# candrewlee14/zgml

Hardware: AMD Instinct MI355X
Metric: decode_tokens_per_sec (higher is better)
Workload: dtype f32; 1 GPU; SmolLM-135M Q4_0 greedy decode, batch 1, 1xMI355X (BASELINE configs[1]); weights=synthetic Q4_0 (int4 + f16 block scale / 32), tied f32 LM head, max_seq=2048, loop=device-resident (inputs in HBM), parallelism=none

## Files before the change

### zgml_amd/csrc/attention_decode.h

```cpp
#pragma once
#include "kernels.h"

#include <hip/hip_fp16.h>
#include <math.h>

namespace zgml {
namespace {

typedef float f4v_t __attribute__((ext_vector_type(4)));
__device__ __forceinline__ float4 ldg4(const float* p) {
    const f4v_t v = *(const __attribute__((address_space(1))) f4v_t*)p;
    return make_float4(v.x, v.y, v.z, v.w);
}
__device__ __forceinline__ float ldg1(const float* p) { return *(const __attribute__((address_space(1))) float*)p; }
__device__ __forceinline__ uint32_t ldgu(const uint32_t* p) { return *(const __attribute__((address_space(1))) uint32_t*)p; }
__device__ __forceinline__ void stg4(float* p, float4 v) { *(__attribute__((address_space(1))) f4v_t*)p = f4v_t{v.x, v.y, v.z, v.w}; }
__device__ __forceinline__ void stg1(float* p, float v) { *(__attribute__((address_space(1))) float*)p = v; }
__device__ __forceinline__ void stgu(uint32_t* p, uint32_t v) { *(__attribute__((address_space(1))) uint32_t*)p = v; }

constexpr int kAttnBlock = 1024;
constexpr int kAttnUnroll = 4;

__device__ __forceinline__ float4 rope4(float4 own, float4 par, float4 c, float4 s, bool is_hi) {
    if (is_hi)
        return make_float4(own.x * c.x + par.x * s.x, own.y * c.y + par.y * s.y, own.z * c.z + par.z * s.z,
                           own.w * c.w + par.w * s.w);
    return make_float4(own.x * c.x - par.x * s.x, own.y * c.y - par.y * s.y, own.z * c.z - par.z * s.z,
                       own.w * c.w - par.w * s.w);
}

__device__ __forceinline__ float score_of(float dot, float mk, float scale) {
    float score = -INFINITY;
    if (isfinite(mk)) {
        score = dot * scale + mk;
        if (!isfinite(score)) score = -INFINITY;
    }
    return score;
}


__device__ __forceinline__ float xor16_sum(float v) {
    auto r = __builtin_amdgcn_permlane16_swap(__float_as_uint(v), __float_as_uint(v), false, false);
    return __uint_as_float(r[0]) + __uint_as_float(r[1]);
}
__device__ __forceinline__ float xor32_sum(float v) {
    auto r = __builtin_amdgcn_permlane32_swap(__float_as_uint(v), __float_as_uint(v), false, false);
    return __uint_as_float(r[0]) + __uint_as_float(r[1]);
}
__device__ __forceinline__ float xor16_max(float v) {
    auto r = __builtin_amdgcn_permlane16_swap(__float_as_uint(v), __float_as_uint(v), false, false);
    return fmaxf(__uint_as_float(r[0]), __uint_as_float(r[1]));
}
__device__ __forceinline__ float xor32_max(float v) {
    auto r = __builtin_amdgcn_permlane32_swap(__float_as_uint(v), __float_as_uint(v), false, false);
    return fmaxf(__uint_as_float(r[0]), __uint_as_float(r[1]));
}

template <int LPK>
__device__ __forceinline__ float group_sum(float v) {
    if (LPK >= 2) v += __int_as_float(__builtin_amdgcn_mov_dpp(__float_as_int(v), 0xB1, 0xF, 0xF, true));
    if (LPK >= 4) v += __int_as_float(__builtin_amdgcn_mov_dpp(__float_as_int(v), 0x4E, 0xF, 0xF, true));
    if (LPK >= 8) v += __int_as_float(__builtin_amdgcn_mov_dpp(__float_as_int(v), 0x141, 0xF, 0xF, true));
    if (LPK >= 16) v += __int_as_float(__builtin_amdgcn_mov_dpp(__float_as_int(v), 0x140, 0xF, 0xF, true));
    if (LPK >= 32) v = xor16_sum(v);
    if (LPK >= 64) v = xor32_sum(v);
    return v;
}

struct SoftState {
    float m, l;
    float4 acc;
};
__device__ __forceinline__ void soft_merge(SoftState& s, float om, float ol, float4 oacc) {
    const float nm = fmaxf(s.m, om);
    const float a = s.m > -INFINITY ? expf(s.m - nm) : 0.0f, b = om > -INFINITY ? expf(om - nm) : 0.0f;
    s.l = s.l * a + ol * b;
    s.acc = make_float4(s.acc.x * a + oacc.x * b, s.acc.y * a + oacc.y * b, s.acc.z * a + oacc.z * b, s.acc.w * a + oacc.w * b);
    s.m = nm;
}

using gu64 = __attribute__((address_space(1))) unsigned long long;
using gu32 = __attribute__((address_space(1))) unsigned int;
__device__ __forceinline__ void split_put(float* p, float a, float b) {
    const unsigned long long v = (unsigned long long)__float_as_uint(a) | ((unsigned long long)__float_as_uint(b) << 32);
    __hip_atomic_store((gu64*)p, v, __ATOMIC_RELAXED, __HIP_MEMORY_SCOPE_AGENT);
// ... 40 lines not shown
__device__ __forceinline__ float row_dot(const float4& q, const AttnRow<false>& r) { return q.x * r.v.x + q.y * r.v.y + q.z * r.v.z + q.w * r.v.w; }
__device__ __forceinline__ float row_dot(const float4& q, const AttnRow<true>& r) {
    const uint32_t kw = r.w;
    return (q.x * (float)(int8_t)(kw & 255) + q.y * (float)(int8_t)((kw >> 8) & 255) + q.z * (float)(int8_t)((kw >> 16) & 255) +
            q.w * (float)(int8_t)(kw >> 24)) * r.sc;
}
__device__ __forceinline__ void row_axpy(float4& acc, float wgt, const AttnRow<false>& r) {
    acc.x += wgt * r.v.x, acc.y += wgt * r.v.y, acc.z += wgt * r.v.z, acc.w += wgt * r.v.w;
}
__device__ __forceinline__ void row_axpy(float4& acc, float wgt, const AttnRow<true>& r) {
    const float ws = wgt * r.sc;
    const uint32_t vw = r.w;
    acc.x += ws * (float)(int8_t)(vw & 255), acc.y += ws * (float)(int8_t)((vw >> 8) & 255);
    acc.z += ws * (float)(int8_t)((vw >> 16) & 255), acc.w += ws * (float)(int8_t)(vw >> 24);
}
__device__ __forceinline__ AttnRow<true> quantise_block32(float4 v) {
    float mx = fmaxf(fmaxf(fabsf(v.x), fabsf(v.y)), fmaxf(fabsf(v.z), fabsf(v.w)));
    mx = fmaxf(mx, __int_as_float(__builtin_amdgcn_mov_dpp(__float_as_int(mx), 0xB1, 0xF, 0xF, true)));
    mx = fmaxf(mx, __int_as_float(__builtin_amdgcn_mov_dpp(__float_as_int(mx), 0x4E, 0xF, 0xF, true)));
    mx = fmaxf(mx, __int_as_float(__builtin_amdgcn_mov_dpp(__float_as_int(mx), 0x141, 0xF, 0xF, true)));
    const float scale = mx > 0.f ? mx / 127.0f : 1.0f, inv = mx > 0.f ? 127.0f / mx : 0.0f;
    auto q8 = [&](float x) { return (uint32_t)(uint8_t)(int8_t)(int)fminf(fmaxf(x * inv, -127.0f), 127.0f); };
    return AttnRow<true>{q8(v.x) | (q8(v.y) << 8) | (q8(v.z) << 16) | (q8(v.w) << 24), scale};
}

#ifndef ZGML_ATTN_KVQ16
#define ZGML_ATTN_KVQ16 1
#endif
constexpr int kAttnUnrollQ16 = 4;
typedef uint32_t u4v_t __attribute__((ext_vector_type(4)));
__device__ __forceinline__ u4v_t ldgu4(const void* p) { return *(const __attribute__((address_space(1))) u4v_t*)p; }
template <int B>
__device__ __forceinline__ float s8_to_f32(uint32_t w) {
    float r;
#if defined(__HIP_DEVICE_COMPILE__)
    if constexpr (B == 0) asm("v_cvt_f32_i32_sdwa %0, sext(%1) dst_sel:DWORD dst_unused:UNUSED_PAD src0_sel:BYTE_0" : "=v"(r) : "v"(w));
    if constexpr (B == 1) asm("v_cvt_f32_i32_sdwa %0, sext(%1) dst_sel:DWORD dst_unused:UNUSED_PAD src0_sel:BYTE_1" : "=v"(r) : "v"(w));
    if constexpr (B == 2) asm("v_cvt_f32_i32_sdwa %0, sext(%1) dst_sel:DWORD dst_unused:UNUSED_PAD src0_sel:BYTE_2" : "=v"(r) : "v"(w));
    if constexpr (B == 3) asm("v_cvt_f32_i32_sdwa %0, sext(%1) dst_sel:DWORD dst_unused:UNUSED_PAD src0_sel:BYTE_3" : "=v"(r) : "v"(w));
#else
    r = (float)(int8_t)(w >> (8 * B));
#endif
    return r;
}
typedef float f32x2_t __attribute__((ext_vector_type(2)));
__device__ __forceinline__ float dot16(const f32x2_t (&q)[8], const u4v_t& w) {
    f32x2_t s = {0.f, 0.f};
#pragma unroll
    for (int c = 0; c < 4; c++) {
        const f32x2_t lo = {s8_to_f32<0>(w[c]), s8_to_f32<1>(w[c])}, hi = {s8_to_f32<2>(w[c]), s8_to_f32<3>(w[c])};
        s = __builtin_elementwise_fma(lo, q[2 * c], s);
        s = __builtin_elementwise_fma(hi, q[2 * c + 1], s);
#if defined(__HIP_DEVICE_COMPILE__)
        __builtin_amdgcn_sched_barrier(0);
#endif
    }
    return s.x + s.y;
}
__device__ __forceinline__ void axpy16(f32x2_t (&acc)[8], float ws, const u4v_t& w) {
    const f32x2_t ws2 = {ws, ws};
#pragma unroll
    for (int c = 0; c < 4; c++) {
        const f32x2_t lo = {s8_to_f32<0>(w[c]), s8_to_f32<1>(w[c])}, hi = {s8_to_f32<2>(w[c]), s8_to_f32<3>(w[c])};
        acc[2 * c] = __builtin_elementwise_fma(lo, ws2, acc[2 * c]);
        acc[2 * c + 1] = __builtin_elementwise_fma(hi, ws2, acc[2 * c + 1]);
#if defined(__HIP_DEVICE_COMPILE__)
        __builtin_amdgcn_sched_barrier(0);
#endif
    }
}
template <int L, bool MAX>
__device__ __forceinline__ float slots_all(float v) {
    auto op = [](float a, float b) { return MAX ? fmaxf(a, b) : a + b; };
    if (L <= 1) v = op(v, __int_as_float(__builtin_amdgcn_mov_dpp(__float_as_int(v), 0x121, 0xF, 0xF, true)));
    if (L <= 2) v = op(v, __int_as_float(__builtin_amdgcn_mov_dpp(__float_as_int(v), 0x122, 0xF, 0xF, true)));
    if (L <= 4) v = op(v, __int_as_float(__builtin_amdgcn_mov_dpp(__float_as_int(v), 0x124, 0xF, 0xF, true)));
    if (L <= 8) v = op(v, __int_as_float(__builtin_amdgcn_mov_dpp(__float_as_int(v), 0x128, 0xF, 0xF, true)));
    if (L <= 16) v = MAX ? xor16_max(v) : xor16_sum(v);
    if (L <= 32) v = MAX ? xor32_max(v) : xor32_sum(v);
    return v;
}

struct DecodeHandoff {
    const uint32_t* cnt;
    uint32_t* seen;
    const uint32_t* idx;
    uint32_t n_heads;
    uint32_t need;
    uint32_t* timeout;
    uint32_t poll_sleep;
};

template <int LPK, bool KVQ, int BLOCK = kAttnBlock>
__device__ __forceinline__ void attention_decode_body(const AttnDecodeParams* __restrict__ params, float* split_buf, uint32_t* split_cnt,
                                                      uint32_t split_min_keys, const uint32_t hx, const uint32_t sp_in, const uint32_t n_sp,
                                                      const DecodeHandoff* ho) {
    constexpr int DH = 4 * LPK, HALF = DH / 2;
    constexpr bool Q16 = KVQ && ZGML_ATTN_KVQ16 != 0 && LPK >= 32;
    constexpr int LPKM = Q16 ? DH / 16 : LPK, KPW = 64 / LPKM, KPW4 = 64 / LPK, U = Q16 ? kAttnUnrollQ16 : kAttnUnroll;
    using Row = AttnRow<KVQ>;
    static_assert(sizeof(AttnDecodeParams) == 248, "the bulk fetch below covers exactly 62 dwords");
    AttnDecodeParams P;
    {
        typedef uint32_t u32x16_t __attribute__((ext_vector_type(16)));
        typedef uint32_t u32x8_t __attribute__((ext_vector_type(8)));
        typedef uint32_t u32x4_t __attribute__((ext_vector_type(4)));
        typedef uint32_t u32x2_t __attribute__((ext_vector_type(2)));
        u32x16_t ra, rb, rc;
        u32x8_t rd;
        u32x4_t re;
        u32x2_t rf;
#if defined(__HIP_DEVICE_COMPILE__)
        const AttnDecodeParams* const rec = params + hx;
        asm volatile("s_load_dwordx16 %0, %6, 0x0\n\ts_load_dwordx16 %1, %6, 0x40\n\ts_load_dwordx16 %2, %6, 0x80\n\t"
                     "s_load_dwordx8 %3, %6, 0xc0\n\ts_load_dwordx4 %4, %6, 0xe0\n\ts_load_dwordx2 %5, %6, 0xf0\n\ts_waitcnt lgkmcnt(0)"
                     : "=&s"(ra), "=&s"(rb), "=&s"(rc), "=&s"(rd), "=&s"(re), "=&s"(rf)
                     : "s"(rec)
                     : "memory");
#else
        ra = rb = rc = u32x16_t{}, rd = u32x8_t{}, re = u32x4_t{}, rf = u32x2_t{};
#endif
        char* const dst = (char*)&P;
        __builtin_memcpy(dst, &ra, 64), __builtin_memcpy(dst + 64, &rb, 64), __builtin_memcpy(dst + 128, &rc, 64);
        __builtin_memcpy(dst + 192, &rd, 32), __builtin_memcpy(dst + 224, &re, 16), __builtin_memcpy(dst + 240, &rf, 8);
    }
    const AttentionParams& p = P.att;
#ifdef ZGML_TRACE
    unsigned long long* const trace = P.trace;
#define ATTN_STAMP(i) do { if (trace && threadIdx.x == 0) trace[i] = wall_clock64(); } while (0)
#else
#define ATTN_STAMP(i) do { } while (0)
#endif
    ATTN_STAMP(0);
    __shared__ __attribute__((aligned(8))) float part_ml[2 * (BLOCK / 64)];
    __shared__ float4 part_acc[(BLOCK / 64) * LPK];
    constexpr int COLV = DH / 4 + DH / 32;
    __shared__ __attribute__((aligned(16))) float q16_lds[Q16 ? DH : 4];
    __shared__ __attribute__((aligned(16))) uint32_t col_lds[Q16 ? 2 * COLV : 4];
    const uint32_t tid = threadIdx.x, lane = tid & 63, w = tid >> 6;
    const uint32_t slot = lane / LPK, li = lane % LPK, d0 = 4 * li, pair = d0 & (HALF - 1);
    const bool is_hi = d0 >= (uint32_t)HALF;
    const uint32_t seq_kv = KVQ ? min(ldgu(p.dyn_seq_kv), P.kvq_cols) : ldgu(p.dyn_seq_kv), dk = ldgu(P.dyn_k_off), dv = ldgu(P.dyn_v_off);
    const uint32_t d2_off = p.dst2 ? ldgu(p.dyn_dst2_off) : 0;
    const bool wait_qkv = ho && ho->cnt;
    float4 q_own, q_par, k_own, k_par, v_new;
    if (!wait_qkv) {
        q_own = ldg4(P.q_src + d0), q_par = ldg4(P.q_src + (d0 ^ HALF));
        k_own = ldg4(P.k_src + d0), k_par = ldg4(P.k_src + (d0 ^ HALF));
        v_new = ldg4(P.v_src + d0);
    }
    const float4 q_c = ldg4(P.q_cs + pair), q_s = ldg4(P.q_cs + HALF + pair);
    const float4 k_c = ldg4(P.k_cs + pair), k_s = ldg4(P.k_cs + HALF + pair);
    ATTN_STAMP(1);
    const uint32_t sp = sp_in;
    uint32_t n_active = 1, k_begin = 0, k_end = seq_kv;
    if (n_sp > 1) {
        n_active = seq_kv / split_min_keys;
        n_active = n_active < 1 ? 1 : (n_active > n_sp ? n_sp : n_active);
        if (sp >= n_active) {
            if (wait_qkv && tid == 0) {
                uint32_t* const seen = ho->seen + (hx * n_sp + sp) * 3;
                seen[0] += ho->need, seen[1] += ho->need, seen[2] += ho->need;
            }
            return;
        }
        const uint32_t chunk = (seq_kv + n_active - 1) / n_active;
        k_begin = min(sp * chunk, seq_kv), k_end = min(k_begin + chunk, seq_kv);
    }
    const uint32_t n_keys = k_end - k_begin;
    constexpr int KEYS_PER_WAVE = Q16 ? KPW : KPW * U;
    uint32_t NW = (n_keys + KEYS_PER_WAVE - 1) / KEYS_PER_WAVE;
    NW = NW < 1 ? 1 : (NW > (uint32_t)(BLOCK / 64) ? (uint32_t)(BLOCK / 64) : NW);
    if (w >= NW) return;
    const uint32_t keys_per_iter = KPW * NW, step_keys = keys_per_iter * U, last = k_end ? k_end - 1 : 0;
    constexpr uint32_t BPC = DH / 32;
    const int8_t* const kq = (const int8_t*)P.k_cache + d0;
    const int8_t* const vq = (const int8_t*)P.v_cache + d0;
    const float* const ksc = P.k_cache + (uint64_t)P.kvq_cols * DH / 4 + d0 / 32;
    const float* const vsc = P.v_cache + (uint64_t)P.kvq_cols * DH / 4 + d0 / 32;
    auto load_k = [&](uint32_t s) -> Row {
        if constexpr (KVQ)
            return Row{ldgu((const uint32_t*)(kq + (uint64_t)s * DH)), ldg1(ksc + (uint64_t)s * BPC)};
        else
            return Row{ldg4(p.k + (uint64_t)s * p.k_cs + d0)};
    };
    auto load_v = [&](uint32_t s) -> Row {
        if constexpr (KVQ)
            return Row{ldgu((const uint32_t*)(vq + (uint64_t)s * DH)), ldg1(vsc + (uint64_t)s * BPC)};
        else
            return Row{ldg4(p.v + (uint64_t)s * p.v_cs + d0)};
    };
    Row kv[Q16 ? 1 : U], vv[Q16 ? 1 : U];
    float mk[U];
    const uint32_t slotm = lane / LPKM, lim = lane % LPKM;
    const char* const kb16 = (const char*)P.k_cache;
    const char* const vb16 = (const char*)P.v_cache;
    const uint32_t sc_base16 = P.kvq_cols * (uint32_t)DH + 4 * (lim / 2);
    u4v_t kw[Q16 ? U : 1], vw[Q16 ? U : 1];
    float ks[Q16 ? U : 1], vs[Q16 ? U : 1];
    auto issue_k16 = [&](uint32_t base) {
#pragma unroll
        for (int j = 0; j < U; j++) {
            const uint32_t s = min(base + j * keys_per_iter + w * KPW + slotm, last);
            kw[j] = ldgu4(kb16 + (s * (uint32_t)DH + 16 * lim));
            ks[j] = ldg1((const float*)(kb16 + (sc_base16 + s * (4 * BPC))));
            mk[j] = ldg1((const float*)((const char*)p.mask + s * (4 * p.mask_rs)));
        }
    };
    auto issue_v16 = [&](uint32_t base) {
#pragma unroll
        for (int j = 0; j < U; j++) {
            const uint32_t s = min(base + j * keys_per_iter + w * KPW + slotm, last);
            vw[j] = ldgu4(vb16 + (s * (uint32_t)DH + 16 * lim));
            vs[j] = ldg1((const float*)(vb16 + (sc_base16 + s * (4 * BPC))));
        }
    };
    if constexpr (Q16) {
        issue_k16(k_begin);
        issue_v16(k_begin);
    } else {
#pragma unroll
        for (int j = 0; j < U; j++) {
            const uint32_t s = min(k_begin + j * keys_per_iter + w * KPW + slot, last);
            kv[j] = load_k(s);
            vv[j] = load_v(s);
            mk[j] = ldg1(p.mask + (uint64_t)s * p.mask_rs);
        }
    }
    uint32_t target[3] = {0, 0, 0};
    if (wait_qkv) {
        const uint32_t ci[3] = {ho->idx[3 * hx], ho->idx[3 * hx + 1], ho->idx[3 * hx + 2]};
        const uint32_t* const seen = ho->seen + (hx * n_sp + sp) * 3;
#pragma unroll
        for (int c = 0; c < 3; c++) target[c] = seen[c] + ho->need;
        if (w == 0) {
            uint32_t spins = 0;
            for (;;) {
                bool ok = true;
#pragma unroll
                for (int c = 0; c < 3; c++)
                    ok = ok && (int32_t)(__hip_atomic_load((gu32*)ho->cnt + 32 * ci[c], __ATOMIC_RELAXED, __HIP_MEMORY_SCOPE_AGENT) - target[c]) >= 0;
                if (ok) break;
                if (++spins > 400000u) {
                    if (tid == 0) __hip_atomic_store(ho->timeout, 1u, __ATOMIC_RELAXED, __HIP_MEMORY_SCOPE_SYSTEM);
                    break;
                }
                for (uint32_t z = 0; z < ho->poll_sleep; z++) __builtin_amdgcn_s_sleep(1);
            }
        }
        __builtin_amdgcn_fence(__ATOMIC_ACQUIRE, "wavefront");
        if (NW > 1) __syncthreads();
        auto ld_agent4 = [](const float* p) {
            float4 v;
            split_get(p, v.x, v.y);
            split_get(p + 2, v.z, v.w);
            return v;
        };
        q_own = ld_agent4(P.q_src + d0), q_par = ld_agent4(P.q_src + (d0 ^ HALF));
        k_own = ld_agent4(P.k_src + d0), k_par = ld_agent4(P.k_src + (d0 ^ HALF));
        v_new = ld_agent4(P.v_src + d0);
    }
    ATTN_STAMP(2);
    const float4 qv = rope4(q_own, q_par, q_c, q_s, is_hi);
    const float4 k_new = rope4(k_own, k_par, k_c, k_s, is_hi);
    uint32_t col_k, col_v;
    Row k_col, v_col;
    if constexpr (KVQ) {
        col_k = dk, col_v = dv;
        k_col = quantise_block32(k_new), v_col = quantise_block32(v_new);
    } else {
        col_k = (dk - P.k_off) / p.k_cs, col_v = (dv - P.v_off) / p.v_cs;
        k_col = Row{k_new}, v_col = Row{v_new};
    }
    if (w == 0 && slot == 0 && sp == 0) {
        stg4(P.q_rot + d0, qv);
        if (P.owner) {
            stg4(P.k_rot + d0, k_new);
            if constexpr (KVQ) {
                if (col_k < P.kvq_cols) {
                    stgu((uint32_t*)((int8_t*)P.k_cache + (uint64_t)col_k * DH + d0), k_col.w);
                    if ((li & 7) == 0) stg1(P.k_cache + (uint64_t)P.kvq_cols * DH / 4 + (uint64_t)col_k * BPC + d0 / 32, k_col.sc);
                }
                if (col_v < P.kvq_cols) {
                    stgu((uint32_t*)((int8_t*)P.v_cache + (uint64_t)col_v * DH + d0), v_col.w);
                    if ((li & 7) == 0) stg1(P.v_cache + (uint64_t)P.kvq_cols * DH / 4 + (uint64_t)col_v * BPC + d0 / 32, v_col.sc);
                }
            } else {
                stg4(P.k_cache + dk + d0, k_new);
                stg4(P.v_cache + dv + d0, v_new);
            }
        }
    }
    ATTN_STAMP(3);
    SoftState st{-INFINITY, 0.f, make_float4(0.f, 0.f, 0.f, 0.f)};
    if constexpr (Q16) {
        if (slot == 0) {
            *(float4*)&q16_lds[d0] = qv;
            col_lds[li] = k_col.w, col_lds[COLV + li] = v_col.w;
            if ((li & 7) == 0) col_lds[DH / 4 + li / 8] = __float_as_uint(k_col.sc), col_lds[COLV + DH / 4 + li / 8] = __float_as_uint(v_col.sc);
        }
        __builtin_amdgcn_fence(__ATOMIC_RELEASE, "wavefront");
        __builtin_amdgcn_wave_barrier();
        __builtin_amdgcn_fence(__ATOMIC_ACQUIRE, "wavefront");
        f32x2_t q16[8], acc16[8];
#pragma unroll
        for (int c = 0; c < 4; c++) {
            const float4 t4 = *(const float4*)&q16_lds[16 * lim + 4 * c];
            q16[2 * c] = f32x2_t{t4.x, t4.y}, q16[2 * c + 1] = f32x2_t{t4.z, t4.w};
        }
        float m16 = -INFINITY, l16 = 0.f;
#pragma unroll
        for (int e = 0; e < 8; e++) acc16[e] = f32x2_t{0.f, 0.f};
        const uint32_t wu = __builtin_amdgcn_readfirstlane(w);
        float sc[U], bm;
        auto scores = [&](uint32_t base) {
            bm = -INFINITY;
#pragma unroll
            for (int j = 0; j < U; j++) {
                sc[j] = -INFINITY;
                if (base + j * keys_per_iter + wu * KPW >= k_end) continue;
                const uint32_t t = base + j * keys_per_iter + w * KPW + slotm;
                u4v_t kk = kw[j];
                float kss = ks[j];
                if (__builtin_amdgcn_ballot_w64(t == col_k) != 0 && t == col_k)
                    kk = *(const u4v_t*)&col_lds[4 * lim], kss = __uint_as_float(col_lds[DH / 4 + lim / 2]);
                const float dot = group_sum<LPKM>(dot16(q16, kk) * kss);
                sc[j] = t < k_end ? score_of(dot, mk[j], p.scale) : -INFINITY;
                bm = fmaxf(bm, sc[j]);
            }
        };
        auto update = [&](uint32_t base) {
            const float nm = fmaxf(m16, bm);
            if (nm > -INFINITY) {
                const float alpha = m16 > -INFINITY ? __expf(m16 - nm) : 0.0f;
                l16 *= alpha;
#pragma unroll
                for (int e = 0; e < 8; e++) acc16[e] *= alpha;
#pragma unroll
                for (int j = 0; j < U; j++) {
                    if (base + j * keys_per_iter + wu * KPW >= k_end) continue;
                    const uint32_t t = base + j * keys_per_iter + w * KPW + slotm;
                    const float wgt = sc[j] > -INFINITY ? __expf(sc[j] - nm) : 0.0f;
                    u4v_t xx = vw[j];
// ... 43 lines not shown
            const uint32_t t = base + j * keys_per_iter + w * KPW + slot;
            const Row kk = t == col_k ? k_col : kv[j];
            const float dot = group_sum<LPK>(row_dot(qv, kk));
            sc[j] = t < k_end ? score_of(dot, mk[j], p.scale) : -INFINITY;
            bm = fmaxf(bm, sc[j]);
        }
        const float nm = fmaxf(st.m, bm);
        if (nm > -INFINITY) {
            const float alpha = st.m > -INFINITY ? expf(st.m - nm) : 0.0f;
            st.l *= alpha;
            st.acc = make_float4(st.acc.x * alpha, st.acc.y * alpha, st.acc.z * alpha, st.acc.w * alpha);
#pragma unroll
            for (int j = 0; j < U; j++) {
                const uint32_t t = base + j * keys_per_iter + w * KPW + slot;
                const float wgt = sc[j] > -INFINITY ? expf(sc[j] - nm) : 0.0f;
                const Row x = t == col_v ? v_col : vv[j];
                st.l += wgt;
                if (sc[j] > -INFINITY) row_axpy(st.acc, wgt, x);
            }
            st.m = nm;
        }
    };
    if (n_keys <= step_keys) {
        if (n_keys) step(k_begin);
    } else {
        for (uint32_t base = k_begin; base < k_end; base += step_keys) {
            Row kn[U], vn[U];
            float mn[U];
#pragma unroll
            for (int j = 0; j < U; j++) {
                const uint32_t s = min(base + step_keys + j * keys_per_iter + w * KPW + slot, last);
                kn[j] = load_k(s);
                vn[j] = load_v(s);
                mn[j] = ldg1(p.mask + (uint64_t)s * p.mask_rs);
            }
            step(base);
#pragma unroll
            for (int j = 0; j < U; j++) kv[j] = kn[j], vv[j] = vn[j], mk[j] = mn[j];
        }
    }
    ATTN_STAMP(4);
    slots_merge<LPK>(st);
    }
    SoftState r = st;
    if (NW > 1) {
        if (!Q16 && lane < LPK) {
            part_acc[w * LPK + lane] = st.acc;
            if (lane == 0) part_ml[2 * w] = st.m, part_ml[2 * w + 1] = st.l;
        }
        ATTN_STAMP(5);
        __syncthreads();
        ATTN_STAMP(6);
        if (w != 0) return;
        constexpr int MAXW = BLOCK / 64, NPS = MAXW / KPW4 > 0 ? MAXW / KPW4 : 1;
        static_assert(MAXW <= 16, "lanes 0..15 (one DPP row) hold the waves' maxima");
        float M = lane < NW ? part_ml[2 * lane] : -INFINITY;
        float2 ml[NPS];
        float4 pa[NPS];
#pragma unroll
        for (int i = 0; i < NPS; i++) {
            const uint32_t ww = slot + i * KPW4, wc = ww < NW ? ww : 0;
            ml[i] = *(const float2*)&part_ml[2 * wc];
            pa[i] = part_acc[wc * LPK + li];
        }
        M = fmaxf(M, __int_as_float(__builtin_amdgcn_mov_dpp(__float_as_int(M), 0xB1, 0xF, 0xF, true)));
        M = fmaxf(M, __int_as_float(__builtin_amdgcn_mov_dpp(__float_as_int(M), 0x4E, 0xF, 0xF, true)));
        M = fmaxf(M, __int_as_float(__builtin_amdgcn_mov_dpp(__float_as_int(M), 0x141, 0xF, 0xF, true)));
        M = fmaxf(M, __int_as_float(__builtin_amdgcn_mov_dpp(__float_as_int(M), 0x140, 0xF, 0xF, true)));
        M = __int_as_float(__builtin_amdgcn_readfirstlane(__float_as_int(M)));
        r = SoftState{M, 0.f, make_float4(0.f, 0.f, 0.f, 0.f)};
#pragma unroll
        for (int i = 0; i < NPS; i++) {
            const bool live = slot + i * KPW4 < NW && ml[i].x > -INFINITY;
            const float f = live ? expf(ml[i].x - M) : 0.0f;
            r.l += ml[i].y * f;
            r.acc.x += pa[i].x * f, r.acc.y += pa[i].y * f, r.acc.z += pa[i].z * f, r.acc.w += pa[i].w * f;
        }
        slots_sum<LPK>(r);
    } else {
        ATTN_STAMP(5);
        ATTN_STAMP(6);
    }
    {
        if (wait_qkv && lane == 0) {
            uint32_t* const seen = ho->seen + (hx * n_sp + sp) * 3;
            seen[0] = target[0], seen[1] = target[1], seen[2] = target[2];
        }
        if (n_active > 1) {
            constexpr uint32_t REC = DH + 4;
            float* const head_buf = split_buf + (uint64_t)hx * n_sp * REC;
            float* const mine = head_buf + (uint64_t)sp * REC;
            if (lane < LPK) {
                if (lane == 0) split_put(mine, r.m, r.l);
                split_put(mine + 4 + 4 * lane, r.acc.x, r.acc.y);
                split_put(mine + 4 + 4 * lane + 2, r.acc.z, r.acc.w);
            }
            asm volatile("s_waitcnt vmcnt(0)" ::: "memory");
            uint32_t old = 0;
            if (lane == 0) old = __hip_atomic_fetch_add((gu32*)(split_cnt + hx), 1u, __ATOMIC_RELAXED, __HIP_MEMORY_SCOPE_AGENT);
            old = __shfl(old, 0, 64);
            if (old != n_active - 1) return;
            __builtin_amdgcn_fence(__ATOMIC_ACQUIRE, "wavefront");
            r = SoftState{-INFINITY, 0.f, make_float4(0.f, 0.f, 0.f, 0.f)};
            for (uint32_t c = slot; c < n_active; c += KPW4) {
                const float* rec = head_buf + (uint64_t)c * REC;
                float om, ol;
                float4 oa;
                split_get(rec, om, ol);
                split_get(rec + 4 + 4 * li, oa.x, oa.y);
                split_get(rec + 4 + 4 * li + 2, oa.z, oa.w);
                soft_merge(r, om, ol, oa);
            }
            slots_merge<LPK>(r);
            if (lane == 0) __hip_atomic_store((gu32*)(split_cnt + hx), 0u, __ATOMIC_RELAXED, __HIP_MEMORY_SCOPE_AGENT);
        }
        if (lane < LPK) {
            const float inv_l = r.l > 0.f ? 1.0f / r.l : 0.0f;
            const float o[4] = {r.acc.x * inv_l, r.acc.y * inv_l, r.acc.z * inv_l, r.acc.w * inv_l};
            stg4(p.dst + 4 * lane, make_float4(o[0], o[1], o[2], o[3]));
            if (p.dst2) {
#pragma unroll
                for (int e = 0; e < 4; e++) stg1(p.dst2 + (uint64_t)d2_off + (uint64_t)(4 * lane + e) * p.d2_rs, o[e]);
            }
        }
    }
    ATTN_STAMP(7);
#undef ATTN_STAMP
}

template <int LPK, bool KVQ, int BLOCK = kAttnBlock>
__global__ void __launch_bounds__(BLOCK) attention_decode_kernel(const AttnDecodeParams* __restrict__ params, float* split_buf,
                                                                 uint32_t* split_cnt, uint32_t split_min_keys) {
    attention_decode_body<LPK, KVQ, BLOCK>(params, split_buf, split_cnt, split_min_keys, blockIdx.x, blockIdx.y, gridDim.y, nullptr);
}

}
}
```

### zgml_amd/csrc/kernels.h

```cpp
#pragma once

#include <hip/hip_runtime.h>
#include <stdint.h>
#include <stdlib.h>

#include "../../include/zgml_hip.h"
#include "sample.h"
#include "switches.h"

namespace zgml {

inline uint32_t device_cus() {
    static const uint32_t n = [] {
        int dev = 0, cus = 0;
        if (hipGetDevice(&dev) != hipSuccess || hipDeviceGetAttribute(&cus, hipDeviceAttributeMultiprocessorCount, dev) != hipSuccess || cus <= 0) cus = 256;
        return (uint32_t)cus;
    }();
    return n;
}

constexpr int kMaxFusedSteps = 8;

struct FusedStepDev {
    uint32_t op;
// ... 417 lines not shown
    uint32_t* picks = nullptr;
    const uint32_t* pos_word = nullptr;
    uint32_t rows_per_seq = 1, pos_stride = 0;
};
struct SampleWindow {
    const uint32_t* list = nullptr;
    uint32_t n_list = 0;
    uint32_t* ring = nullptr;
    const uint32_t* lo = nullptr;
    const uint32_t* hist = nullptr;
    const uint32_t* cand = nullptr;
    const uint32_t* lo_word = nullptr;
    uint32_t hist_stride = 0;
};
struct SampleConstraintRow {
    const uint16_t* class_of;
    const uint16_t* next;
    uint32_t n_classes, con_active;
    const uint32_t* forced;
};
struct SampleConstraint {
    const SampleConstraintRow* rows = nullptr;
    uint32_t* state = nullptr;
};
inline size_t sample_scratch_keys(uint64_t n, uint32_t rows) { return (size_t)rows * sample_slices(n) * 256; }
inline uint32_t sample_merge_keys(uint32_t slices, uint32_t run) {
    uint32_t P = run;
    while (P < slices * run) P <<= 1;
    return P;
}
enum SampledSel { kSelPlain, kSelPenalized, kSelConstrained, kSelConstrainedRows, kSampledSels };
void launch_sample(hipStream_t s, const float* v, uint64_t n, uint32_t rows, uint64_t* scratch, const SampleParamsDev* params, const SampleAdvance& adv,
                   SampledSel sel = kSelPlain, const SampleWindow& win = SampleWindow{}, const SampleConstraint& con = SampleConstraint{});
void launch_logprob(hipStream_t s, const float* v, uint64_t n, uint32_t rows, float* part);
struct LogprobTarget {
    float* out = nullptr;
    const uint32_t* tokens = nullptr;
    const int64_t* token64 = nullptr;
    const uint32_t* picks = nullptr;
    const uint32_t* state = nullptr;
    const int64_t* emitted = nullptr;
    uint32_t* written = nullptr;
    uint32_t cap = 0, n_seqs = 0;
};
void launch_logprob_finish(hipStream_t s, const float* v, uint64_t n, uint32_t rows, const float* part, const LogprobTarget& t);
void launch_sample_select(hipStream_t s, const float* v, uint64_t n, uint32_t rows, uint64_t* scratch);
struct TopLogprobTarget {
    LogprobTarget chosen;
    uint32_t* top_tok = nullptr;
    float* top_val = nullptr;
    const SampleParamsDev* params = nullptr;
    uint32_t shared_params = 0, top_n = 0;
};
void launch_logprob_finish_top(hipStream_t s, const float* v, uint64_t n, uint32_t rows, const float* part, const uint64_t* lists, const TopLogprobTarget& t);
void launch_copy_f4(hipStream_t s, void* dst, const void* src, uint64_t bytes);
void launch_f32_to_f16(hipStream_t s, void* dst, const float* src, uint64_t n);

uint32_t classify_qweight(hipStream_t s, const int8_t* raw_data, uint64_t n_elems, const float* raw_scales,
                          uint64_t n_blocks, uint32_t* flag_scratch );
void launch_pack_gguf(hipStream_t s, const uint8_t* raw_blocks, const QWeightDev& out);
bool qweight_packable(uint64_t K, uint64_t N, uint64_t bs);
bool w8a8_applies(uint64_t K, uint64_t N, uint64_t bs);
void w8a8_packed_bytes(uint64_t K, uint64_t N, uint64_t* qs_bytes, uint64_t* sc_bytes);
void launch_pack_w8a8(hipStream_t s, const int8_t* raw_data, const float* raw_scales, const QWeightDev& out);
void launch_w8a8_matvec(hipStream_t s, const QWeightDev& w, const float* x, float* dst);
void packed_bytes(QWFormat format, uint32_t scale_f16, uint64_t K, uint64_t N, uint64_t* qs_bytes,
                  uint64_t* sc_bytes);
void launch_pack_qweight(hipStream_t s, const int8_t* raw_data, const float* raw_scales, const QWeightDev& out);
constexpr uint64_t kQmmScratchHead = 16384;
constexpr uint64_t kQmmCounterBytes = 4096;
uint64_t qmatmul_scratch_bytes(const QWeightDev& w, uint32_t M);
void launch_qmatmul(hipStream_t s, const QWeightDev& w, const QMatmulParams& p, float* scratch);
constexpr uint32_t kKonRowsMaxM = 8;
constexpr uint32_t kKonRowsRoutedM = 6;
bool launch_qmatvec_kon_rows(hipStream_t s, const QWeightDev& w, const QMatmulParams& p);
bool qmatmul_can_group(const QWeightDev& a, const QMatmulParams& pa, const QWeightDev& b, const QMatmulParams& pb);
uint32_t qmatmul_max_group();
void launch_qmatmul_group(hipStream_t s, const QWeightDev* w, const QMatmulParams* p, uint32_t n, float* scratch);
bool qmv_prenorm_ok(const QWeightDev& w, uint32_t K, uint64_t total_cols, uint32_t M);
bool qmv_pair_ok(const QWeightDev& w);
bool qmv_can_group(const QWeightDev& a, const QWeightDev& b);
uint32_t qmv_max_prologue_k(const QWeightDev& w);
void launch_qmatvec_fused(hipStream_t s, const QmvLaunch& L);
bool launch_qkv_attention(hipStream_t s, const QmvLaunch& L, const AttnDecodeParams* dev_params, uint32_t n_heads, uint32_t n_kv, uint32_t d_head,
                          const AttnSplit& sp, uint32_t* counters, const uint32_t* idx, uint32_t* seen, uint32_t* timeout,
                          bool kvq = false);
int qkv_attn_kon_census(hipStream_t s, uint32_t d_head, bool kvq, uint32_t grid);
int qkv_attn_kon_blocks_per_cu(uint32_t d_head, bool kvq);
void launch_synth_packed(hipStream_t s, const QWeightDev& w, uint32_t matrix_id);

struct KsVec {
    const float* base = nullptr;
    const float* parts = nullptr;
    uint32_t n_parts = 0;
    float* sum_dst = nullptr;
    float* add_dst = nullptr;
};
struct KsNormIn {
    KsVec x;
    const float* gamma = nullptr;
    float eps = 0.f;
    float* store_mid = nullptr;
    float* store_x = nullptr;
    uint32_t K = 0;
};
struct KsProjLaunch {
    KsNormIn in;
    uint32_t n_parts = 0;
    QWeightDev w[3];
    float* dst[3] = {nullptr, nullptr, nullptr};
    unsigned long long* trace = nullptr;
};
struct KsAttnOLaunch {
    const AttnDecodeParams* dev = nullptr;
    uint32_t n_heads = 0, d_head = 0;
    AttnSplit sp;
    bool kvq = false;
    QWeightDev wo;
    float* parts_out = nullptr;
    uint8_t head_of[64] = {0};
    unsigned long long* trace = nullptr;
};
struct KsMlpLaunch {
    KsNormIn in;
    QWeightDev gate, up, down;
    float *gate_out = nullptr, *up_out = nullptr, *exp_out = nullptr, *silu_out = nullptr, *prod_out = nullptr;
    const float* ones = nullptr;
    float* parts_out = nullptr;
    unsigned long long* trace = nullptr;
};
bool ks_weight_ok(const QWeightDev& w);
bool ks_proj_ok(const KsProjLaunch& L);
bool ks_attn_o_ok(const KsAttnOLaunch& L);
bool ks_mlp_ok(const KsMlpLaunch& L);
bool ks_norm_ok(const KsNormIn& in);
uint32_t ks_mlp_parts(const KsMlpLaunch& L);
bool ks_layer_a_ok(const KsProjLaunch& PL, const KsAttnOLaunch& AL);
uint32_t ks_layer_a_proj_wgs(const KsProjLaunch& PL);
bool launch_ks_layer_a(hipStream_t s, const KsProjLaunch& PL, const KsAttnOLaunch& AL, uint32_t n_kv, uint32_t* counters, const uint32_t* idx, uint32_t* seen,
                       uint32_t* timeout);
void launch_ks_proj(hipStream_t s, const KsProjLaunch& L);
void launch_ks_attn_o(hipStream_t s, const KsAttnOLaunch& L);
void launch_ks_mlp(hipStream_t s, const KsMlpLaunch& L);
void launch_ks_norm(hipStream_t s, const KsNormIn& in);

struct PeerGatherArgs {
    char* const* blocks;
    float* local;
    uint32_t* seen;
    uint32_t* timeout;
    uint64_t ctr_off, stage_off;
    uint64_t wait_ticks;
    uint32_t len, rank, world;
    uint64_t poison_off;
};
struct PeerArgmaxArgs {
    char* const* blocks;
    const float* slice;
    uint32_t* seen;
    uint32_t* timeout;
    int64_t* out;
    uint64_t ctr_off, pairs_off, wait_ticks;
    uint32_t len, rank, world;
    uint64_t poison_off;
};
void launch_peer_gather(hipStream_t s, const PeerGatherArgs& a);
void launch_peer_argmax(hipStream_t s, const PeerArgmaxArgs& a);
void launch_local_argmax_pair(hipStream_t s, const float* slice, uint32_t len, uint32_t rank, unsigned long long* pairs);
void launch_reduce_pairs(hipStream_t s, const unsigned long long* pairs, uint32_t world, int64_t* out);
// ... 3 lines not shown
```

### zgml_amd/csrc/ksplit.hip

```cpp
#include "qmv_common.h"
#include "attention_decode.h"

#include <hip/hip_fp16.h>
#include <math.h>
#include <stdio.h>
#include <stdlib.h>

namespace zgml {

namespace {

struct KsUnit {
    uint4 wq;
    uint32_t s2;
};
__device__ __forceinline__ KsUnit ks_load(const uint4* qs, const uint32_t* sc, uint32_t KC, uint32_t g, uint32_t c, uint32_t i) {
    KsUnit u;
    u.wq = qs[((uint64_t)g * KC + c) * 16 + i];
    u.s2 = sc[((uint64_t)(g >> 1) * KC + c) * 16 + i];
    return u;
}
__device__ __forceinline__ void ks_fma(const KsUnit& u, float xa, float xb, bool ok, float& a0, float& a1, float& a2, float& a3) {
    const __half2 h = *(const __half2*)&u.s2;
    float tA = ok ? (__low2float(h) * 16.0f) * xa : 0.f;
// ... 97 lines not shown
            for (uint32_t j = 0; j < kFly; j++) {
                const uint32_t p = p0 + j * S;
                v[j] = ldg4(in.x.parts + (uint64_t)(p < P ? p : p0) * K + 4 * q);
            }
#pragma unroll
            for (uint32_t j = 0; j < kFly; j++)
                if (p0 + j * S < P) a = add4(a, v[j]);
        }
        if (act) l.sl[s * Q + q] = a;
        KS_STAMP(tr, 2);
        ks_barrier();
        float4 sv[16];
        sum = l.sl[qc];
        if (S <= 16) {
#pragma unroll
            for (uint32_t s2 = 1; s2 < 16; s2++) sv[s2] = l.sl[(s2 < S ? s2 : 0) * Q + qc];
#pragma unroll
            for (uint32_t s2 = 1; s2 < 16; s2++)
                if (s2 < S) sum = add4(sum, sv[s2]);
        } else {
            for (uint32_t s2 = 1; s2 < S; s2++) sum = add4(sum, l.sl[s2 * Q + qc]);
        }
        h = add4(sum, base4);
    }
    if (store && mine && P) {
        if (in.x.sum_dst) stg4(in.x.sum_dst + 4 * tid, sum);
        if (in.x.add_dst) stg4(in.x.add_dst + 4 * tid, h);
    }
    KS_STAMP(tr, 3);
    if (mine) *(float4*)(l.xs + 4 * tid) = make_float4(h.x * g4.x, h.y * g4.y, h.z * g4.z, h.w * g4.w);
    for (uint32_t z = Q + tid; z < KC * 8; z += T) *(float4*)(l.xs + 4 * z) = make_float4(0.f, 0.f, 0.f, 0.f);
    if (in.gamma) {
        const float ss = rows_sum4(row16_sum(mine ? (h.x * h.x + h.y * h.y) + (h.z * h.z + h.w * h.w) : 0.f));
        if ((tid & 63) == 0) l.red[tid >> 6] = ss;
    }
    ks_barrier();
    KS_STAMP(tr, 4);
    if (store && in.gamma) {
        const float inv = ks_inv(in, l.red, T);
        if (mine) {
            const float4 mid = make_float4(h.x * inv, h.y * inv, h.z * inv, h.w * inv);
            if (in.store_mid) stg4(in.store_mid + 4 * tid, mid);
            if (in.store_x) stg4(in.store_x + 4 * tid, make_float4(mid.x * g4.x, mid.y * g4.y, mid.z * g4.z, mid.w * g4.w));
        }
    }
}

template <int U>
__device__ __forceinline__ void ks_row_load(KsUnit (&u)[U], const uint4* qs, const uint32_t* sc, uint32_t KC, uint32_t g, uint32_t slot, uint32_t n_slots, uint32_t i) {
#pragma unroll
    for (int j = 0; j < U; j++) {
        const uint32_t c = slot + j * n_slots;
        u[j] = ks_load(qs, sc, KC, g, c < KC ? c : KC - 1, i);
    }
}
template <int U>
__device__ __forceinline__ float ks_row_fma(const KsUnit (&u)[U], const float* xs, uint32_t KC, uint32_t slot, uint32_t n_slots, uint32_t i) {
    float a0 = 0.f, a1 = 0.f, a2 = 0.f, a3 = 0.f;
#pragma unroll
    for (int j = 0; j < U; j++) {
        const uint32_t c = slot + j * n_slots;
        const bool ok = c < KC;
        const uint32_t cc = ok ? c : KC - 1;
        ks_fma(u[j], xs[cc * 32 + i], xs[cc * 32 + 16 + i], ok, a0, a1, a2, a3);
    }
    return (a0 + a1) + (a2 + a3);
}

struct KsProjArgs {
    KsNormIn in;
    const uint4* qs[3];
    const uint32_t* sc[3];
    float* out[3];
    uint32_t wg_begin[3];
    uint32_t n_parts, KC;
    unsigned long long* trace;
    uint32_t n_threads;
};
struct KsPublish {
    uint32_t* cnt;
    uint32_t base[3];
    uint32_t groups_shift;
};
template <int GP, int U>
__device__ __forceinline__ void ks_proj_body(const KsProjArgs& a, float* smem, const KsPublish* pub) {
    const uint32_t T = a.n_threads ? a.n_threads : blockDim.x, W = T >> 6, b = blockIdx.x;
    if (threadIdx.x >= T) return;
    const uint32_t lane = threadIdx.x & 63, w = threadIdx.x >> 6, r = lane >> 4, i = lane & 15;
#define KS_T T
    KS_STAMPS(ts, a.trace, blockIdx.x == 0);
#undef KS_T
    KS_STAMP(ts, 0);
    uint32_t pi = 0;
    if (a.n_parts > 1 && b >= a.wg_begin[1]) pi = 1;
    if (a.n_parts > 2 && b >= a.wg_begin[2]) pi = 2;
    const uint4* const qs = pi == 2 ? a.qs[2] : pi == 1 ? a.qs[1] : a.qs[0];
    const uint32_t* const sc = pi == 2 ? a.sc[2] : pi == 1 ? a.sc[1] : a.sc[0];
    float* const out = pi == 2 ? a.out[2] : pi == 1 ? a.out[1] : a.out[0];
    const uint32_t g0 = (b - (pi == 2 ? a.wg_begin[2] : pi == 1 ? a.wg_begin[1] : 0u)) * GP;
    const uint32_t rho = 4 * w + r, combo = r % GP, slot = rho / GP, n_slots = 4 * W / GP, g = g0 + combo;
    KsUnit u[U];
    const KsLds l = ks_lds(smem, a.KC, T);
    ks_prologue(a.in, l, a.KC, T, b == 0, ts, [&]() {
        ks_row_load<U>(u, qs, sc, a.KC, g, slot, n_slots, i);
        KS_STAMP(ts, 1);
    });
    float v = ks_row_fma<U>(u, l.xs, a.KC, slot, n_slots, i);
    KS_STAMP(ts, 5);
    if (GP == 1) v = rows_sum4(v);
    if (GP == 2) v = xor32_sum(v);
    if (r < (uint32_t)GP) l.red2[(w * GP + r) * 16 + i] = v;
    ks_barrier();
    KS_STAMP(ts, 6);
    if (w == 0) {
      const float inv = ks_inv(a.in, l.red, T);
      if (r < (uint32_t)GP) {
        float pw[16], t = 0.f;
#pragma unroll
        for (uint32_t ww = 0; ww < 16; ww++) pw[ww] = l.red2[((ww < W ? ww : 0) * GP + r) * 16 + i];
#pragma unroll
        for (uint32_t ww = 0; ww < 16; ww++)
            if (ww < W) t += pw[ww];
        if (pub)
            __hip_atomic_store((__attribute__((address_space(1))) float*)out + (g0 + r) * 16 + i, t * inv, __ATOMIC_RELAXED, __HIP_MEMORY_SCOPE_AGENT);
        else
            out[(g0 + r) * 16 + i] = t * inv;
      }
      if (pub) {
#if defined(__HIP_DEVICE_COMPILE__)
        asm volatile("s_waitcnt vmcnt(0)" ::: "memory");
#endif
        if (lane == 0)
            __hip_atomic_fetch_add((__attribute__((address_space(1))) uint32_t*)pub->cnt + 32 * (pub->base[pi] + (g0 >> pub->groups_shift)), 1u, __ATOMIC_RELAXED,
                                   __HIP_MEMORY_SCOPE_AGENT);
      }
    }
    KS_STAMP(ts, 7);
    KS_FLUSH(ts, a.trace);
}
template <int GP, int U>
__global__ void __launch_bounds__(1024) ks_proj_kernel(KsProjArgs a) {
    extern __shared__ __attribute__((aligned(16))) float smem[];
    ks_proj_body<GP, U>(a, smem, nullptr);
}

struct KsMlpArgs {
    KsNormIn in;
    const uint4 *qs_g, *qs_u, *qs_d;
    const uint32_t *sc_g, *sc_u, *sc_d;
    uint32_t KC;
    uint32_t NB2_d;
    uint32_t KC_d;
    float *gate_out, *up_out, *exp_out, *silu_out, *prod_out;
    const float* ones;
    float* parts_out;
    unsigned long long* trace;
};
template <int UG, int UD>
__global__ void __launch_bounds__(1024) ks_mlp_kernel(KsMlpArgs a) {
    extern __shared__ __attribute__((aligned(16))) float smem[];
    const uint32_t T = blockDim.x, W = T >> 6, R = 4 * W, b = blockIdx.x;
    const uint32_t lane = threadIdx.x & 63, w = threadIdx.x >> 6, r = lane >> 4, i = lane & 15, rho = 4 * w + r;
#define KS_T blockDim.x
    KS_STAMPS(ts, a.trace, blockIdx.x == 0);
    KS_STAMP(ts, 0);
    const uint4* const qs = (r >> 1) ? a.qs_u : a.qs_g;
    const uint32_t* const sc = (r >> 1) ? a.sc_u : a.sc_g;
    KsUnit ug[UG], ud[UD];
    const uint32_t n = 32 * b + (lane & 31);
    float ones = 0.f;
    const KsLds l = ks_lds(smem, a.KC, T);
    ks_prologue(a.in, l, a.KC, T, b == 0, ts, [&]() {
        ks_row_load<UG>(ug, qs, sc, a.KC, 2 * b + (r & 1), w, W, i);
#pragma unroll
        for (int j = 0; j < UD; j++) {
            const uint32_t gd = rho + j * R;
            ud[j] = ks_load(a.qs_d, a.sc_d, a.KC_d, gd < a.NB2_d ? gd : a.NB2_d - 1, b, i);
        }
        ones = a.ones[n];
        KS_STAMP(ts, 1);
    });
    const float acc = ks_row_fma<UG>(ug, l.xs, a.KC, w, W, i);
    KS_STAMP(ts, 5);
    l.red2[(w * 4 + r) * 16 + i] = acc;
    ks_barrier();
    KS_STAMP(ts, 6);
    if (w == 0) {
        const float inv = ks_inv(a.in, l.red, T);
        float pw[16], v = 0.f;
#pragma unroll
        for (uint32_t ww = 0; ww < 16; ww++) pw[ww] = l.red2[((ww < W ? ww : 0) * 4 + r) * 16 + i];
#pragma unroll
        for (uint32_t ww = 0; ww < 16; ww++)
            if (ww < W) v += pw[ww];
        v *= inv;
        const float other = __shfl_xor(v, 32, 64);
        if (lane < 32) {
            const float gate = v, up = other;
            a.gate_out[n] = gate;
            a.up_out[n] = up;
            const float e = expf(-gate);
            a.exp_out[n] = e;
            const float sl = (1.0f / (e + ones)) * gate;
            a.silu_out[n] = sl;
            const float pr = sl * up;
            a.prod_out[n] = pr;
            l.su[lane] = pr;
        }
        KS_STAMP(ts, 7);
    }
    ks_barrier();
    KS_STAMP(ts, 8);
    const float xa = l.su[i], xb = l.su[16 + i];
#pragma unroll
    for (int j = 0; j < UD; j++) {
        const uint32_t gd = rho + j * R;
        const bool ok = gd < a.NB2_d;
        float a0 = 0.f, a1 = 0.f, a2 = 0.f, a3 = 0.f;
        ks_fma(ud[j], xa, xb, ok, a0, a1, a2, a3);
        if (ok) a.parts_out[(uint64_t)b * (16 * a.NB2_d) + gd * 16 + i] = (a0 + a1) + (a2 + a3);
    }
    KS_STAMP(ts, 9);
    KS_FLUSH(ts, a.trace);
}

__global__ void __launch_bounds__(1024) ks_norm_kernel(KsNormIn in, uint32_t KC) {
    extern __shared__ __attribute__((aligned(16))) float smem[];
    const KsLds l = ks_lds(smem, KC, blockDim.x);
    KS_STAMPS(ts, (unsigned long long*)nullptr, false);
    ks_prologue(in, l, KC, blockDim.x, true, ts, []() {});
}

struct KsAttnArgs {
    const AttnDecodeParams* params;
    float* split_buf;
    uint32_t* split_cnt;
    uint32_t split_min_keys, n_sp;
    const uint4* qs_o;
    const uint32_t* sc_o;
    uint32_t KC_o, NB2_o;
    float* parts_out;
    unsigned long long* trace;
    uint8_t head_of[64];
};
constexpr int kKsAttnBlock = 768;
template <int LPK, bool KVQ, int UO>
__device__ __forceinline__ void ks_attn_o_body(const KsAttnArgs& f, const uint32_t hx, const uint32_t sp, const DecodeHandoff* ho) {
    constexpr int DH = 4 * LPK, KPW = 64 / LPK, U = kAttnUnroll, HALF = DH / 2, CH = DH / 32, BLOCK = kKsAttnBlock;
    static_assert(DH % 32 == 0, "the head's rows of W_o are whole 32-k chunks");
    using Row = AttnRow<KVQ>;
    const uint32_t n_sp = f.n_sp;
    KS_STAMPS(ts, f.trace, hx == 0 && sp == 0);
    KS_STAMP(ts, 0);
    const uint32_t head = f.head_of[hx], c_o = head * CH;
    const uint32_t r16 = (threadIdx.x & 63) >> 4, i16 = threadIdx.x & 15, rho = 4 * (threadIdx.x >> 6) + r16;
    KsUnit uo[UO][CH];
#pragma unroll
    for (int j = 0; j < UO; j++) {
        const uint32_t gd = rho + j * (BLOCK / 16);
        const uint32_t gc = gd < f.NB2_o ? gd : f.NB2_o - 1;
#pragma unroll
        for (int c = 0; c < CH; c++) uo[j][c] = ks_load(f.qs_o, f.sc_o, f.KC_o, gc, c_o + c, i16);
    }
    static_assert(sizeof(AttnDecodeParams) == 248, "the bulk fetch below covers exactly 62 dwords");
    AttnDecodeParams P;
    {
        typedef uint32_t u32x16_t __attribute__((ext_vector_type(16)));
        typedef uint32_t u32x8_t __attribute__((ext_vector_type(8)));
        typedef uint32_t u32x4_t __attribute__((ext_vector_type(4)));
        typedef uint32_t u32x2_t __attribute__((ext_vector_type(2)));
        u32x16_t ra, rb, rc;
        u32x8_t rd;
        u32x4_t re;
        u32x2_t rf;
#if defined(__HIP_DEVICE_COMPILE__)
        const AttnDecodeParams* const rec = f.params + hx;
        asm volatile("s_load_dwordx16 %0, %6, 0x0\n\ts_load_dwordx16 %1, %6, 0x40\n\ts_load_dwordx16 %2, %6, 0x80\n\t"
                     "s_load_dwordx8 %3, %6, 0xc0\n\ts_load_dwordx4 %4, %6, 0xe0\n\ts_load_dwordx2 %5, %6, 0xf0\n\ts_waitcnt lgkmcnt(0)"
                     : "=&s"(ra), "=&s"(rb), "=&s"(rc), "=&s"(rd), "=&s"(re), "=&s"(rf)
                     : "s"(rec)
                     : "memory");
#else
        ra = rb = rc = u32x16_t{}, rd = u32x8_t{}, re = u32x4_t{}, rf = u32x2_t{};
#endif
        char* const dst = (char*)&P;
        __builtin_memcpy(dst, &ra, 64), __builtin_memcpy(dst + 64, &rb, 64), __builtin_memcpy(dst + 128, &rc, 64);
        __builtin_memcpy(dst + 192, &rd, 32), __builtin_memcpy(dst + 224, &re, 16), __builtin_memcpy(dst + 240, &rf, 8);
    }
    const AttentionParams& p = P.att;
    KS_STAMP(ts, 1);
    __shared__ __attribute__((aligned(8))) float part_ml[2 * (BLOCK / 64)];
    __shared__ float4 part_acc[(BLOCK / 64) * LPK];
    __shared__ __attribute__((aligned(16))) float o_lds[DH];
    __shared__ uint32_t last_flag;
    const uint32_t tid = threadIdx.x, lane = tid & 63, w = tid >> 6;
    const uint32_t slot = lane / LPK, li = lane % LPK, d0 = 4 * li, pair = d0 & (HALF - 1);
    const bool is_hi = d0 >= (uint32_t)HALF;
    const uint32_t seq_kv = KVQ ? min(ldgu(p.dyn_seq_kv), P.kvq_cols) : ldgu(p.dyn_seq_kv), dk = ldgu(P.dyn_k_off), dv = ldgu(P.dyn_v_off);
    const uint32_t d2_off = head * DH;
    float4 q_own, q_par, k_own, k_par, v_new;
    if (!ho) {
        q_own = ldg4(P.q_src + d0), q_par = ldg4(P.q_src + (d0 ^ HALF));
        k_own = ldg4(P.k_src + d0), k_par = ldg4(P.k_src + (d0 ^ HALF));
        v_new = ldg4(P.v_src + d0);
    }
    const float4 q_c = ldg4(P.q_cs + pair), q_s = ldg4(P.q_cs + HALF + pair);
    const float4 k_c = ldg4(P.k_cs + pair), k_s = ldg4(P.k_cs + HALF + pair);
    uint32_t n_active = 1, k_begin = 0, k_end = seq_kv;
    if (n_sp > 1) {
        n_active = seq_kv / f.split_min_keys;
        n_active = n_active < 1 ? 1 : (n_active > n_sp ? n_sp : n_active);
        if (sp >= n_active) {
            if (ho && tid == 0) {
                uint32_t* const seen = ho->seen + (hx * n_sp + sp) * 3;
                seen[0] += ho->need, seen[1] += ho->need, seen[2] += ho->need;
            }
            return;
        }
        const uint32_t chunk = (seq_kv + n_active - 1) / n_active;
        k_begin = min(sp * chunk, seq_kv), k_end = min(k_begin + chunk, seq_kv);
    }
    const uint32_t n_keys = k_end - k_begin;
    uint32_t NW = (n_keys + KPW * U - 1) / (KPW * U);
    NW = NW < 1 ? 1 : (NW > (uint32_t)(BLOCK / 64) ? (uint32_t)(BLOCK / 64) : NW);
    const uint32_t keys_per_iter = KPW * NW, step_keys = keys_per_iter * U, last = k_end ? k_end - 1 : 0;
    constexpr uint32_t BPC = DH / 32;
    const int8_t* const kq = (const int8_t*)P.k_cache + d0;
    const int8_t* const vq = (const int8_t*)P.v_cache + d0;
    const float* const ksc = P.k_cache + (uint64_t)P.kvq_cols * DH / 4 + d0 / 32;
    const float* const vsc = P.v_cache + (uint64_t)P.kvq_cols * DH / 4 + d0 / 32;
// ... 158 lines not shown
                pa[q] = part_acc[wc * LPK + li];
            }
            M = fmaxf(M, __int_as_float(__builtin_amdgcn_mov_dpp(__float_as_int(M), 0xB1, 0xF, 0xF, true)));
            M = fmaxf(M, __int_as_float(__builtin_amdgcn_mov_dpp(__float_as_int(M), 0x4E, 0xF, 0xF, true)));
            M = fmaxf(M, __int_as_float(__builtin_amdgcn_mov_dpp(__float_as_int(M), 0x141, 0xF, 0xF, true)));
            M = fmaxf(M, __int_as_float(__builtin_amdgcn_mov_dpp(__float_as_int(M), 0x140, 0xF, 0xF, true)));
            M = __int_as_float(__builtin_amdgcn_readfirstlane(__float_as_int(M)));
            r = SoftState{M, 0.f, make_float4(0.f, 0.f, 0.f, 0.f)};
#pragma unroll
            for (int q = 0; q < NPS; q++) {
                const bool live = slot + q * KPW < NW && ml[q].x > -INFINITY;
                const float fct = live ? expf(ml[q].x - M) : 0.0f;
                r.l += ml[q].y * fct;
                r.acc.x += pa[q].x * fct, r.acc.y += pa[q].y * fct, r.acc.z += pa[q].z * fct, r.acc.w += pa[q].w * fct;
            }
            slots_sum<LPK>(r);
        }
        bool is_last = true;
        if (n_active > 1) {
            constexpr uint32_t REC = DH + 4;
            float* const head_buf = f.split_buf + (uint64_t)hx * n_sp * REC;
            float* const mine = head_buf + (uint64_t)sp * REC;
            if (lane < LPK) {
                if (lane == 0) split_put(mine, r.m, r.l);
                split_put(mine + 4 + 4 * lane, r.acc.x, r.acc.y);
                split_put(mine + 4 + 4 * lane + 2, r.acc.z, r.acc.w);
            }
            asm volatile("s_waitcnt vmcnt(0)" ::: "memory");
            uint32_t old = 0;
            if (lane == 0) old = __hip_atomic_fetch_add((gu32*)(f.split_cnt + hx), 1u, __ATOMIC_RELAXED, __HIP_MEMORY_SCOPE_AGENT);
            old = __shfl(old, 0, 64);
            is_last = old == n_active - 1;
            if (is_last) {
                __builtin_amdgcn_fence(__ATOMIC_ACQUIRE, "wavefront");
                r = SoftState{-INFINITY, 0.f, make_float4(0.f, 0.f, 0.f, 0.f)};
                for (uint32_t c = slot; c < n_active; c += KPW) {
                    const float* rec = head_buf + (uint64_t)c * REC;
                    float om, ol;
                    float4 oa;
                    split_get(rec, om, ol);
                    split_get(rec + 4 + 4 * li, oa.x, oa.y);
                    split_get(rec + 4 + 4 * li + 2, oa.z, oa.w);
                    soft_merge(r, om, ol, oa);
                }
                slots_merge<LPK>(r);
                if (lane == 0) __hip_atomic_store((gu32*)(f.split_cnt + hx), 0u, __ATOMIC_RELAXED, __HIP_MEMORY_SCOPE_AGENT);
            }
        }
        if (is_last && lane < LPK) {
            const float inv_l = r.l > 0.f ? 1.0f / r.l : 0.0f;
            const float4 o = make_float4(r.acc.x * inv_l, r.acc.y * inv_l, r.acc.z * inv_l, r.acc.w * inv_l);
            stg4(p.dst + 4 * lane, o);
            float* const d2 = p.dst2 + (uint64_t)d2_off + 4 * lane;
            stg4(d2, o);
            *(float4*)(o_lds + 4 * lane) = o;
        }
        if (lane == 0) last_flag = is_last ? 1u : 0u;
    }
    KS_STAMP(ts, 4);
    ks_barrier();
    if (!last_flag) return;
    if (4 * w >= f.NB2_o) return;
#pragma unroll
    for (int j = 0; j < UO; j++) {
        const uint32_t gd = rho + j * (BLOCK / 16);
        const bool ok = gd < f.NB2_o;
        float a0 = 0.f, a1 = 0.f, a2 = 0.f, a3 = 0.f;
#pragma unroll
        for (int c = 0; c < CH; c++) ks_fma(uo[j][c], o_lds[32 * c + i16], o_lds[32 * c + 16 + i16], ok, a0, a1, a2, a3);
        if (ok) f.parts_out[(uint64_t)head * (16 * f.NB2_o) + gd * 16 + i16] = (a0 + a1) + (a2 + a3);
    }
    KS_STAMP(ts, 5);
    KS_FLUSH(ts, f.trace);
}
template <int LPK, bool KVQ, int UO>
__global__ void __launch_bounds__(kKsAttnBlock) ks_attn_o_kernel(KsAttnArgs f) {
    ks_attn_o_body<LPK, KVQ, UO>(f, blockIdx.x, blockIdx.y, nullptr);
}

struct KsLayerAArgs {
    KsProjArgs pj;
    KsAttnArgs at;
    KsPublish pub;
    DecodeHandoff ho;
    uint32_t n_proj, n_heads;
    uint32_t dbg;
};
template <int LPK, bool KVQ, int UO, int GP, int U>
__global__ void __launch_bounds__(kKsAttnBlock) ks_layer_a_kernel(KsLayerAArgs g) {
    extern __shared__ __attribute__((aligned(16))) float smem[];
    if (blockIdx.x < g.n_proj) {
        ks_proj_body<GP, U>(g.pj, smem, &g.pub);
    } else {
        const uint32_t b = blockIdx.x - g.n_proj;
#ifdef ZGML_TRACE
        if (g.dbg == 1) return;
        if (g.dbg == 2) {
            ks_attn_o_body<LPK, KVQ, UO>(g.at, b % g.n_heads, b / g.n_heads, nullptr);
            return;
        }
#endif
        ks_attn_o_body<LPK, KVQ, UO>(g.at, b % g.n_heads, b / g.n_heads, &g.ho);
    }
}

uint32_t ks_pick_waves(uint32_t K, uint32_t rows_wanted) {
    uint32_t W = cdiv(rows_wanted, 4);
    const uint32_t w_min = cdiv(K / 4, 64);
    W = W < w_min ? w_min : W;
    W = W < 1 ? 1 : (W > 16 ? 16 : W);
    return W;
}

bool ks_vec_aligned(const KsNormIn& in) {
    auto a16 = [](const void* p) { return ((uintptr_t)p % 16) == 0; };
    return in.K && in.K % 4 == 0 && in.K / 4 <= 1024 && a16(in.x.base) && a16(in.x.parts) && a16(in.x.sum_dst) && a16(in.x.add_dst) && a16(in.gamma) &&
           a16(in.store_mid) && a16(in.store_x) && (in.x.n_parts == 0 || in.x.parts) && in.x.base;
}

}

bool ks_weight_ok(const QWeightDev& w) { return w.format == QW_Q4 && w.scale_f16 && !w.stream_nt && w.K <= 2048 && w.N % 32 == 0 && w.KC == (w.K + 31) / 32; }

bool ks_norm_ok(const KsNormIn& in) { return ks_vec_aligned(in); }

static uint32_t ks_proj_gp(const KsProjLaunch& L) {
    const int env = sw().ks_proj_gp;
    uint32_t gp = env == 1 || env == 2 || env == 4 ? (uint32_t)env : 2u;
    for (uint32_t t = 0; t < L.n_parts; t++)
        while (gp > 1 && (L.w[t].N / 16) % gp) gp >>= 1;
    return gp;
}

bool ks_proj_ok(const KsProjLaunch& L) {
    if (L.n_parts < 1 || L.n_parts > 3 || !ks_vec_aligned(L.in) || !L.in.gamma) return false;
    for (uint32_t t = 0; t < L.n_parts; t++)
        if (!ks_weight_ok(L.w[t]) || L.w[t].K != L.in.K || !L.dst[t]) return false;
    return true;
}

void launch_ks_proj(hipStream_t s, const KsProjLaunch& L) {
    const uint32_t gp = ks_proj_gp(L), KC = L.w[0].KC;
    KsProjArgs a{};
    a.in = L.in, a.n_parts = L.n_parts, a.KC = KC, a.trace = L.trace;
    uint32_t wgs = 0;
    for (uint32_t t = 0; t < 3; t++) {
        const uint32_t tt = t < L.n_parts ? t : 0;
        a.qs[t] = (const uint4*)L.w[tt].qs, a.sc[t] = (const uint32_t*)L.w[tt].sc, a.out[t] = L.dst[tt];
        a.wg_begin[t] = wgs;
        if (t < L.n_parts) wgs += (uint32_t)(L.w[t].N / 16) / gp;
    }
    const int env_w = sw().ks_proj_waves;
    uint32_t W = ks_pick_waves(L.in.K, KC * gp);
    if (env_w >= 1 && env_w <= 16 && (uint32_t)env_w * 64 >= L.in.K / 4) W = (uint32_t)env_w;
    const uint32_t n_slots = 4 * W / gp, U = cdiv(KC, n_slots);
    const size_t lds = ks_lds_bytes(KC, W * 64);
    using Fn = void (*)(KsProjArgs);
    Fn fn = nullptr;
#define KS_PROJ(G) (U <= 1 ? (Fn)ks_proj_kernel<G, 1> : U <= 2 ? (Fn)ks_proj_kernel<G, 2> : U <= 4 ? (Fn)ks_proj_kernel<G, 4> : (Fn)ks_proj_kernel<G, 8>)
    fn = gp == 4 ? KS_PROJ(4) : gp == 2 ? KS_PROJ(2) : KS_PROJ(1);
#undef KS_PROJ
    if (U > 8) {
        fprintf(stderr, "[zgml_hip] ERROR: ks_proj: %u units per row: not launched\n", U);
        return;
    }
    hipLaunchKernelGGL(fn, dim3(wgs), dim3(W * 64), lds, s, a);
}
// ... 4 lines not shown
    const uint32_t KC = L.gate.KC, NB2_d = (uint32_t)(L.down.N / 16);
    const int env_w = sw().ks_mlp_waves;
    W = ks_pick_waves(L.in.K, std::max(NB2_d, 2 * KC));
    if (env_w >= 1 && env_w <= 16 && (uint32_t)env_w * 64 >= L.in.K / 4) W = (uint32_t)env_w;
    UG = cdiv(KC, W), UD = cdiv(NB2_d, 4 * W);
}

bool ks_mlp_ok(const KsMlpLaunch& L) {
    if (!ks_vec_aligned(L.in) || !L.in.gamma || !ks_weight_ok(L.gate) || !ks_weight_ok(L.up) || !ks_weight_ok(L.down)) return false;
    if (L.gate.K != L.in.K || L.up.K != L.in.K || L.gate.N != L.up.N || L.down.K != L.gate.N || L.down.K % 32) return false;
    if (!L.gate_out || !L.up_out || !L.exp_out || !L.silu_out || !L.prod_out || !L.ones || !L.parts_out) return false;
    uint32_t W, UG, UD;
    ks_mlp_shape(L, W, UG, UD);
    return UG <= 4 && UD <= 2;
}

void launch_ks_mlp(hipStream_t s, const KsMlpLaunch& L) {
    uint32_t W, UG, UD;
    ks_mlp_shape(L, W, UG, UD);
    KsMlpArgs a{};
    a.in = L.in;
    a.qs_g = (const uint4*)L.gate.qs, a.qs_u = (const uint4*)L.up.qs, a.qs_d = (const uint4*)L.down.qs;
    a.sc_g = (const uint32_t*)L.gate.sc, a.sc_u = (const uint32_t*)L.up.sc, a.sc_d = (const uint32_t*)L.down.sc;
    a.KC = L.gate.KC, a.NB2_d = (uint32_t)(L.down.N / 16), a.KC_d = L.down.KC;
    a.gate_out = L.gate_out, a.up_out = L.up_out, a.exp_out = L.exp_out, a.silu_out = L.silu_out, a.prod_out = L.prod_out;
    a.ones = L.ones, a.parts_out = L.parts_out, a.trace = L.trace;
    using Fn = void (*)(KsMlpArgs);
    Fn fn = nullptr;
#define KS_MLP(D) (UG <= 1 ? (Fn)ks_mlp_kernel<1, D> : UG <= 2 ? (Fn)ks_mlp_kernel<2, D> : UG <= 3 ? (Fn)ks_mlp_kernel<3, D> : (Fn)ks_mlp_kernel<4, D>)
    fn = UD <= 1 ? KS_MLP(1) : KS_MLP(2);
#undef KS_MLP
    if (UG > 4 || UD > 2) {
        fprintf(stderr, "[zgml_hip] ERROR: ks_mlp: shape outside the kernel's unit counts: not launched\n");
        return;
    }
    hipLaunchKernelGGL(fn, dim3(ks_mlp_parts(L)), dim3(W * 64), ks_lds_bytes(a.KC, W * 64), s, a);
}

void launch_ks_norm(hipStream_t s, const KsNormIn& in) {
    const uint32_t KC = (in.K + 31) / 32, W = ks_pick_waves(in.K, std::min<uint32_t>(in.x.n_parts + 1, 16) * cdiv(in.K / 4, 64) * 4);
    hipLaunchKernelGGL(ks_norm_kernel, dim3(1), dim3(W * 64), ks_lds_bytes(KC, W * 64), s, in, KC);
}

static bool ks_layer_a_shape(const KsProjLaunch& PL, const KsAttnOLaunch& AL, uint32_t& U, uint32_t& UO) {
    if (ks_proj_gp(PL) != 2 || PL.n_parts != 3) return false;
    const uint32_t W = kKsAttnBlock / 64;
    if ((uint32_t)W * 64 < PL.in.K / 4) return false;
    const uint32_t Wp = std::min(W, ks_pick_waves(PL.in.K, PL.w[0].KC * 2));
    U = cdiv(PL.w[0].KC, 4 * Wp / 2), UO = cdiv((uint32_t)(AL.wo.N / 16), kKsAttnBlock / 16);
    return U <= 2 && UO <= 2 && (AL.d_head / 16) % 2 == 0;
}
bool ks_layer_a_ok(const KsProjLaunch& PL, const KsAttnOLaunch& AL) {
    uint32_t U, UO;
    return ks_proj_ok(PL) && ks_attn_o_ok(AL) && ks_layer_a_shape(PL, AL, U, UO);
}
uint32_t ks_layer_a_proj_wgs(const KsProjLaunch& PL) {
    uint32_t wgs = 0;
    for (uint32_t t = 0; t < PL.n_parts; t++) wgs += (uint32_t)(PL.w[t].N / 16) / 2;
    return wgs;
}
bool launch_ks_layer_a(hipStream_t s, const KsProjLaunch& PL, const KsAttnOLaunch& AL, uint32_t n_kv, uint32_t* counters, const uint32_t* idx, uint32_t* seen,
                       uint32_t* timeout) {
    uint32_t U, UO;
    if (!ks_layer_a_shape(PL, AL, U, UO)) return false;
    KsLayerAArgs g{};
    KsProjArgs& a = g.pj;
    a.in = PL.in, a.n_parts = PL.n_parts, a.KC = PL.w[0].KC, a.trace = PL.trace;
    a.n_threads = 64 * std::min<uint32_t>(kKsAttnBlock / 64, ks_pick_waves(PL.in.K, PL.w[0].KC * 2));
    uint32_t wgs = 0;
    for (uint32_t t = 0; t < 3; t++) {
        a.qs[t] = (const uint4*)PL.w[t].qs, a.sc[t] = (const uint32_t*)PL.w[t].sc, a.out[t] = PL.dst[t];
        a.wg_begin[t] = wgs;
        wgs += (uint32_t)(PL.w[t].N / 16) / 2;
    }
    KsAttnArgs& f = g.at;
    f.params = AL.dev, f.split_buf = AL.sp.buf, f.split_cnt = AL.sp.cnt, f.split_min_keys = AL.sp.min_keys;
    f.n_sp = AL.sp.splits ? AL.sp.splits : 1;
    f.qs_o = (const uint4*)AL.wo.qs, f.sc_o = (const uint32_t*)AL.wo.sc, f.KC_o = AL.wo.KC, f.NB2_o = (uint32_t)(AL.wo.N / 16);
    f.parts_out = AL.parts_out, f.trace = AL.trace;
    for (uint32_t h = 0; h < 64; h++) f.head_of[h] = AL.head_of[h];
    uint32_t shift = 0;
    while ((16u << shift) < AL.d_head) shift++;
    g.pub = KsPublish{counters, {0, AL.n_heads, AL.n_heads + n_kv}, shift};
    g.ho = DecodeHandoff{counters, seen, idx, AL.n_heads, (AL.d_head / 16) / 2, timeout, (uint32_t)sw().hip_handoff_sleep};
    g.n_proj = wgs, g.n_heads = AL.n_heads;
    g.dbg = (uint32_t)sw().ks_debug_a;
    using Fn = void (*)(KsLayerAArgs);
    Fn fn = nullptr;
#define KS_LA2(LPK_, KVQ_, UO_) (U <= 1 ? (Fn)ks_layer_a_kernel<LPK_, KVQ_, UO_, 2, 1> : (Fn)ks_layer_a_kernel<LPK_, KVQ_, UO_, 2, 2>)
#define KS_LA(LPK_, KVQ_) (UO <= 1 ? KS_LA2(LPK_, KVQ_, 1) : KS_LA2(LPK_, KVQ_, 2))
    if (AL.d_head == 64)
        fn = AL.kvq ? KS_LA(16, true) : KS_LA(16, false);
    else
        fn = AL.kvq ? KS_LA(32, true) : KS_LA(32, false);
#undef KS_LA
#undef KS_LA2
    hipLaunchKernelGGL(fn, dim3(wgs + AL.n_heads * f.n_sp), dim3(kKsAttnBlock), ks_lds_bytes(a.KC, kKsAttnBlock), s, g);
    return true;
}

bool ks_attn_o_ok(const KsAttnOLaunch& L) {
    if (!L.dev || !L.n_heads || L.n_heads > 64 || (L.d_head != 64 && L.d_head != 128) || !ks_weight_ok(L.wo) || L.wo.K != (uint64_t)L.n_heads * L.d_head || !L.parts_out) return false;
    return cdiv(L.wo.N / 16, kKsAttnBlock / 16) <= 4;
}

void launch_ks_attn_o(hipStream_t s, const KsAttnOLaunch& L) {
    KsAttnArgs f{};
    f.params = L.dev, f.split_buf = L.sp.buf, f.split_cnt = L.sp.cnt, f.split_min_keys = L.sp.min_keys;
    f.n_sp = L.sp.splits ? L.sp.splits : 1;
    f.qs_o = (const uint4*)L.wo.qs, f.sc_o = (const uint32_t*)L.wo.sc, f.KC_o = L.wo.KC, f.NB2_o = (uint32_t)(L.wo.N / 16);
    f.parts_out = L.parts_out, f.trace = L.trace;
    for (uint32_t h = 0; h < 64; h++) f.head_of[h] = L.head_of[h];
    const uint32_t UO = cdiv(f.NB2_o, kKsAttnBlock / 16);
    const dim3 grid(L.n_heads, f.n_sp);
    using Fn = void (*)(KsAttnArgs);
    Fn fn = nullptr;
#define KS_ATT(LPK_, KVQ_) (UO <= 1 ? (Fn)ks_attn_o_kernel<LPK_, KVQ_, 1> : UO <= 2 ? (Fn)ks_attn_o_kernel<LPK_, KVQ_, 2> : (Fn)ks_attn_o_kernel<LPK_, KVQ_, 4>)
    if (L.d_head == 64)
        fn = L.kvq ? KS_ATT(16, true) : KS_ATT(16, false);
    else
        fn = L.kvq ? KS_ATT(32, true) : KS_ATT(32, false);
#undef KS_ATT
    hipLaunchKernelGGL(fn, grid, dim3(kKsAttnBlock), 0, s, f);
}

}
```

### zgml_amd/csrc/plan.hip

```cpp
#include "runtime_internal.h"

namespace {

float* buf_at(zgml_hip_program* p, uint16_t idx, uint64_t off) { return p->bufs[idx] + off; }

template <typename T>
const T* upload_params(zgml_hip_program* p, const std::vector<T>& v) {
    void* d = nullptr;
    if (hipMalloc(&d, v.size() * sizeof(T)) != hipSuccess) {
        p->ctx->fail("plan: parameter array allocation failed");
        return nullptr;
    }
    if (h2d_sync(p->ctx->stream, d, v.data(), v.size() * sizeof(T)) != hipSuccess) p->ctx->fail("plan: parameter array upload failed");
    p->param_blobs.push_back(d);
    return (const T*)d;
}

AttnSplit attn_split_for(zgml_hip_program* p, uint32_t n_heads, uint32_t d_head, uint32_t max_kv, int default_min_keys = 128) {
    const int want = sw().hip_attn_split;
    const int min_keys_env = sw().hip_attn_split_min_keys;
    AttnSplit sp;
    const int64_t min_keys = p->ctx->opt_attn_split_min_keys >= 0 ? p->ctx->opt_attn_split_min_keys : (min_keys_env >= 0 ? min_keys_env : default_min_keys);
    if (min_keys == 0 || want <= 1) return sp;
    sp.min_keys = (uint32_t)std::min<int64_t>(std::max<int64_t>(32, min_keys), 1 << 30);
// ... 477 lines not shown
}

bool barrier_between_launches(const zgml_hip_program* p, size_t i) {
    const Launch &a = p->plan[i], &b = p->plan[i + 1];
    return barrier_between(p->barriers, std::min(a.op_lo, b.op_lo), std::max(a.op_hi, b.op_hi));
}

unsigned long long* mapped_trace(size_t words) {
    unsigned long long* t = nullptr;
    if (hipHostMalloc((void**)&t, words * sizeof(unsigned long long), hipHostMallocMapped) != hipSuccess) return nullptr;
    memset(t, 0, words * sizeof(unsigned long long));
    return t;
}

void add_access(OpAccess& dst, const OpAccess& src) {
    dst.reads.insert(dst.reads.end(), src.reads.begin(), src.reads.end());
    dst.writes.insert(dst.writes.end(), src.writes.begin(), src.writes.end());
}

bool anchor_ok(zgml_hip_program* p, uint32_t i) {
    const zgml_device_op& op = p->ops[i];
    if (op.kind != ZGML_DOP_QMATMUL || op.u.qmatmul.M != 1) return false;
    const QWeightDev& w = p->qweights[op.u.qmatmul.weight_idx];
    return w.format != QW_RAW && w.format != QW_W8A8 && (op.u.qmatmul.input_offset % 4) == 0;
}

void fuse_qkv_attention(zgml_hip_program* p) {
    if (!sw().hip_fuse_qkv_attn || p->ctx->fuse_qkv_off || !p->ctx->handoff_flag_dev) return;
    const uint64_t resident_cap = p->ctx->opt_fuse_resident_wgs >= 0 ? (uint64_t)p->ctx->opt_fuse_resident_wgs : (uint64_t)std::max(p->ctx->n_cu, 1);
    for (size_t i = 0; i + 1 < p->plan.size(); i++) {
        const auto qd = p->plan[i].qmv_desc;
        const auto ad = p->plan[i + 1].adec_desc;
        if (!qd || !ad) continue;
        const QmvLaunch& L = *qd;
        if (barrier_between_launches(p, i)) continue;
        const bool kon = L.parts[0].w.format == QW_Q4K && L.K > 2048;
        if (L.n_parts != 3 || (L.K > 2048 && !(kon && sw().hip_fuse_qkv_attn_kon)) || L.pro.kind == QMV_PRO_NONE || (ad->dh != 64 && ad->dh != 128) || L.trace) continue;
        if (kon && L.pro.kind != QMV_PRO_PRENORM) continue;
        const bool kvq = ad->kvq;
        bool ok = true;
        for (uint32_t t = 0; t < 3; t++) ok = ok && L.parts[t].n_epi == 0 && (L.parts[t].w.format == QW_Q4 || L.parts[t].w.format == QW_Q4K) && L.parts[t].w.scale_f16;
        const uint32_t nh = ad->nh, dh = ad->dh;
        ok = ok && (uint64_t)nh * dh == L.parts[0].w.N && L.parts[1].w.N == L.parts[2].w.N && L.parts[1].w.N % dh == 0;
        const uint32_t n_kv = ok ? (uint32_t)(L.parts[1].w.N / dh) : 0;
        ok = ok && n_kv != 0 && nh % n_kv == 0;
        std::vector<uint32_t> idx(3 * (size_t)nh);
        std::vector<char> head_seen(nh, 0);
        for (uint32_t r = 0; ok && r < nh; r++) {
            const AttnDecodeParams& a = ad->host[r];
            const ptrdiff_t qo = a.q_src - L.parts[0].dst, ko = a.k_src - L.parts[1].dst, vo = a.v_src - L.parts[2].dst;
            ok = qo >= 0 && qo % dh == 0 && (uint64_t)qo < (uint64_t)nh * dh && ko >= 0 && ko % dh == 0 && (uint64_t)ko < (uint64_t)n_kv * dh && vo == ko &&
                 a.kvq_block == (kvq ? 32u : 0u);
            if (!ok) break;
            const uint32_t h = (uint32_t)(qo / dh), kvh = (uint32_t)(ko / dh);
            ok = !head_seen[h] && kvh == h / (nh / n_kv);
            head_seen[h] = 1;
            idx[3 * r] = h, idx[3 * r + 1] = nh + kvh, idx[3 * r + 2] = nh + n_kv + kvh;
        }
        if (!ok) continue;
        uint32_t n_sp = ad->sp.splits ? ad->sp.splits : 1;
        uint64_t n_mv = 0;
        for (uint32_t t = 0; t < 3; t++) n_mv += L.parts[t].w.N / 16;
        uint64_t cap = resident_cap;
        if (kon && p->ctx->opt_fuse_resident_wgs < 0) {
            const int per_cu = qkv_attn_kon_blocks_per_cu(ad->dh, kvq);
            cap = per_cu > 0 ? (uint64_t)per_cu * (uint64_t)std::max(p->ctx->n_cu, 1) * (uint64_t)sw().hip_fuse_kon_cap_eighths / 8 : 0;
        }
        if (n_mv + nh > cap) continue;
        if (kon && p->ctx->opt_fuse_resident_wgs < 0 && (cap - n_mv) / nh < n_sp) continue;
        n_sp = (uint32_t)std::min<uint64_t>(n_sp, (cap - n_mv) / nh);
        for (uint32_t t = 0; kon && t < 3; t++) ok = ok && L.parts[t].w.format == QW_Q4K;
        if (!ok) continue;
        if (kon && p->ctx->opt_fuse_resident_wgs < 0) {
            const uint32_t grid = (uint32_t)(n_mv + (uint64_t)nh * n_sp);
            const uint64_t key = ((uint64_t)ad->dh << 40) | ((uint64_t)(kvq ? 1 : 0) << 32) | grid;
            auto it = p->ctx->census.find(key);
            if (it == p->ctx->census.end()) {
                const int r = sw().hip_fuse_census ? qkv_attn_kon_census(p->ctx->stream, ad->dh, kvq, grid) : -1;
                it = p->ctx->census.emplace(key, r).first;
                if (r == 0) fprintf(stderr, "[zgml_hip] the fused q/k/v + attention launch of %u workgroups is NOT co-resident on this device (census): two launches instead\n", grid);
            }
            if (it->second == 0) continue;
        }
        const size_t n_cnt = 32 * ((size_t)nh + 2 * n_kv);
        const size_t words = n_cnt + (size_t)nh * n_sp * 3 + 1 + 3 * (size_t)nh;
        uint32_t* block = nullptr;
        if (hipMalloc((void**)&block, words * 4) != hipSuccess) continue;
        if (memset_sync(p->ctx->stream, block, 0, words * 4) != hipSuccess) {
            hipFree(block);
            continue;
        }
        p->fuse_owned.push_back(block);
        uint32_t *counters = block, *seen = block + n_cnt, *timeout = p->ctx->handoff_flag_dev, *idx_dev = seen + (size_t)nh * n_sp * 3 + 1;
        if (h2d_sync(p->ctx->stream, idx_dev, idx.data(), idx.size() * 4) != hipSuccess) continue;
        const AttnDecodeParams* d = ad->dev;
        AttnSplit sp = ad->sp;
        sp.splits = n_sp;
        const uint32_t n_ops = p->plan[i].n_ops + p->plan[i + 1].n_ops, lo = std::min(p->plan[i].op_lo, p->plan[i + 1].op_lo),
                       hi = std::max(p->plan[i].op_hi, p->plan[i + 1].op_hi);
        Launch F{ZGML_DOP_QMATMUL, n_ops, lo, hi, [=](hipStream_t s) {
                     if (!launch_qkv_attention(s, L, d, nh, n_kv, dh, sp, counters, idx_dev, seen, timeout, kvq)) {
                         launch_qmatvec_fused(s, L);
                         launch_attention_decode_batch(s, d, nh, dh, sp, kvq);
                     }
                 }};
        p->plan[i] = std::move(F);
        p->plan.erase(p->plan.begin() + (ptrdiff_t)i + 1);
    }
}

void fuse_ksplit(zgml_hip_program* p) {
    p->has_deferred = false;
    if (!p->ksplit || p->ksplit_off || !p->barriers.empty()) return;
    auto overlap = [](const float* a, size_t na, const float* b, size_t nb) { return a && b && a < b + nb && b < a + na; };
    auto residual_epi = [](const QmvPart& pt) {
        return pt.n_epi == 1 && pt.epi[0].op == ZGML_OP_ADD && pt.epi[0].operand && pt.epi[0].operand != pt.dst && pt.epi[0].store && pt.epi[0].store != pt.dst;
    };
    auto norm_in_safe = [&](const KsNormIn& in) {
        const size_t K = in.K;
        const float* outs[4] = {in.x.sum_dst, in.x.add_dst, in.store_mid, in.store_x};
        for (const float* o : outs) {
            if (!o) continue;
            if (overlap(o, K, in.x.base, K) || overlap(o, K, in.gamma, K) || overlap(o, K, in.x.parts, K * in.x.n_parts)) return false;
            for (const float* o2 : outs)
                if (o2 && o2 != o && overlap(o, K, o2, K)) return false;
        }
        return true;
    };
    std::vector<Launch> out;
    KsVec pend{};
    uint32_t pend_K = 0;
    bool have_pend = false;
    uint32_t pend_lo = 0, pend_hi = 0;
    auto flush = [&]() {
        if (!have_pend) return;
        KsNormIn in;
        in.x = pend, in.K = pend_K;
        Launch M{ZGML_DOP_ELEMENTWISE, 0, pend_lo, pend_hi, [in](hipStream_t s) { launch_ks_norm(s, in); }};
        M.tag = "ks-materialise";
        out.push_back(std::move(M));
        have_pend = false;
    };
    float *parts_o = nullptr, *parts_d = nullptr;
    size_t parts_o_n = 0, parts_d_n = 0;
    auto grow_parts = [&](float*& blk, size_t& have, size_t want) -> bool {
        if (have >= want) return true;
        float* nb = nullptr;
        if (hipMalloc((void**)&nb, want * sizeof(float)) != hipSuccess || memset_sync(p->ctx->stream, nb, 0, want * sizeof(float)) != hipSuccess) {
            if (nb) hipFree(nb);
            return false;
        }
        p->fuse_owned.push_back(nb);
        blk = nb, have = want;
        return true;
    };
    std::vector<Launch>& plan = p->plan;
    size_t i = 0;
    uint32_t n_fused = 0;
    auto new_trace = [&](const char* what) -> unsigned long long* {
        unsigned long long* t = nullptr;
        if (!sw().hip_ks_trace || p->ks_traces.size() >= 24 || !(t = mapped_trace(32))) return nullptr;
        p->ks_traces.push_back({t, what});
        return t;
    };
    while (i < plan.size()) {
        if (i + 2 < plan.size() && plan[i].qmv_desc && plan[i + 1].adec_desc && plan[i + 2].qmv_desc) {
            const QmvLaunch &Q = *plan[i].qmv_desc, &O = *plan[i + 2].qmv_desc;
            const AdecDesc& A = *plan[i + 1].adec_desc;
            bool ok = Q.n_parts == 3 && Q.pro.kind == QMV_PRO_RMSNORM_MUL && !Q.trace && !O.trace && O.n_parts == 1 && O.pro.kind == QMV_PRO_NONE && residual_epi(O.parts[0]) &&
                      !O.next.xg_out && (A.dh == 64 || A.dh == 128) && O.K == A.nh * A.dh && ks_weight_ok(O.parts[0].w);
            for (uint32_t t = 0; ok && t < 3; t++) ok = Q.parts[t].n_epi == 0 && ks_weight_ok(Q.parts[t].w);
            std::vector<char> seen_head(A.nh, 0);
            uint8_t head_of[64] = {0};
            ok = ok && A.nh <= 64;
            for (uint32_t r = 0; ok && r < A.nh; r++) {
                const AttnDecodeParams& a = A.host[r];
                ok = a.att.dst2 == O.pro.a && a.att.d2_rs == 1 && a.att.dyn_dst2_off >= p->dyn_dev && a.att.dyn_dst2_off < p->dyn_dev + p->ops.size() && a.att.dst_rs == 1 &&
                     ((uintptr_t)a.att.dst2 % 16) == 0;
                if (!ok) break;
                const zgml_device_op& so = p->ops[(size_t)(a.att.dyn_dst2_off - p->dyn_dev)];
                ok = so.kind == ZGML_DOP_SLICE_ASSIGN && so.u.slice_assign.patch_stride == 0 && so.u.slice_assign.dst_offset % A.dh == 0 &&
                     so.u.slice_assign.dst_offset / A.dh < A.nh && !seen_head[so.u.slice_assign.dst_offset / A.dh];
                if (ok) seen_head[so.u.slice_assign.dst_offset / A.dh] = 1, head_of[r] = (uint8_t)(so.u.slice_assign.dst_offset / A.dh);
            }
// ... 1053 lines not shown
```

### zgml_amd/csrc/qmatvec.hip

```cpp
#include "qmv_common.h"
#include "attention_decode.h"

#include <hip/hip_fp16.h>
#include <math.h>
#include <stdlib.h>
#include <string.h>

#include <type_traits>
#include <utility>

namespace zgml {

namespace {



struct QMVPartDev {
    const uint4* qs;
    const void* sc;
    float* out;
    uint32_t NB2;
    uint32_t block_begin;
    uint32_t out_rs;
    uint32_t n_epi;
// ... 47 lines not shown
            v = scale4(v, inv);
            if (owner && pro.store_mid && i < K) {
                if (i + 3 < K) *(float4*)(pro.store_mid + i) = v;
                else { pro.store_mid[i] = v.x; if (i + 1 < K) pro.store_mid[i + 1] = v.y; if (i + 2 < K) pro.store_mid[i + 2] = v.z; }
            }
        }
        if (PRO) {
            v = mul4(v, zero_tail(rb.v[j], i, K));
            if (owner && pro.store_x && i < K) {
                if (i + 3 < K) *(float4*)(pro.store_x + i) = v;
                else { pro.store_x[i] = v.x; if (i + 1 < K) pro.store_x[i + 1] = v.y; if (i + 2 < K) pro.store_x[i + 2] = v.z; }
            }
        }
        *(float4*)(xs + (i < k_count ? i : k_count)) = v;
    }
    if (!PRO)
        for (uint32_t i = (threadIdx.x + kXRegs * bdim) * 4; i < k_count; i += bdim * 4)
            *(float4*)(xs + i) = zero_tail(load_x4<XVEC>(xa_row, i, K), i, K);
}

__device__ __forceinline__ void run_epilogue_silu(const QMVPartDev& part, uint32_t n, float raw, float ones) {
    const float e = expf(-raw);
    part.epi[1].store[n] = e;
    const float s = 1.0f / (e + ones);
    part.epi[4].store[n] = s * raw;
}


__device__ __forceinline__ float block_sumsq(const XRegs& r, uint32_t K, float* red, uint32_t bdim) {
    float ss = 0.f;
#pragma unroll
    for (int j = 0; j < kXRegs; j++) {
        const uint32_t i = (threadIdx.x + j * bdim) * 4;
        const float4 v = zero_tail(r.v[j], i, K);
        ss += v.x * v.x;
        ss += v.y * v.y;
        ss += v.z * v.z;
        ss += v.w * v.w;
    }
    return block_total(ss, red, bdim);
}

__device__ __forceinline__ float epi_unary(uint32_t op, float a) {
    switch (op) {
        case ZGML_OP_NEG: return -a;
        case ZGML_OP_ABS: return fabsf(a);
        case ZGML_OP_SGN: return a > 0.f ? 1.f : (a < 0.f ? -1.f : 0.f);
        case ZGML_OP_STEP: return a > 0.f ? 1.f : 0.f;
        case ZGML_OP_RELU: return fmaxf(a, 0.f);
        case ZGML_OP_SQRT: return sqrtf(a);
        case ZGML_OP_RECIP: return 1.0f / a;
        case ZGML_OP_EXP: return expf(a);
        case ZGML_OP_LOG: return logf(a);
        case ZGML_OP_GELU: {
            const float kk = 0.7978845608f * (a + 0.044715f * a * a * a);
            return 0.5f * a * (1.0f + tanhf(kk));
        }
        default: return a;
    }
}


__device__ __forceinline__ void run_epilogue(const QMVPartDev& part, uint32_t n, float v, const float* out_row, float pre0 = 0.f,
                                             bool have_pre0 = false) {
    const float raw = v;
#pragma unroll
    for (uint32_t e = 0; e < (uint32_t)kMaxEpiSteps; e++) {
        if (e >= part.n_epi) break;
        const QmvEpiStep st = part.epi[e];
        if (st.op == ZGML_OP_ADD) {
            const float o = st.operand == out_row ? raw : (e == 0 && have_pre0 ? pre0 : st.operand[n]);
            v = st.swapped ? o + v : v + o;
        } else if (st.op == ZGML_OP_MUL) {
            const float o = st.operand == out_row ? raw : (e == 0 && have_pre0 ? pre0 : st.operand[n]);
            v = st.swapped ? o * v : v * o;
        } else {
            v = epi_unary(st.op, v);
        }
        if (st.store) st.store[n] = v;
    }
}

struct QmvPublish {
    uint32_t* cnt;
    uint32_t base[3];
    uint32_t groups_shift;
    uint32_t drop;
};

struct KonTail {
    float post;
    bool norm;
    float eps;
    uint32_t K;
    float a_s, b_s;
    uint32_t k0, slice;
    bool has_pro;
    bool prenorm;
    float pp[4];
    bool inv_known = false;
    float inv_pre = 1.0f;
};
__device__ __forceinline__ float prenorm_factor(const float (&pp)[4], uint32_t K, float eps) {
    const float ss = rows_sum4(row16_sum((pp[0] + pp[1]) + (pp[2] + pp[3])));
    return 1.0f / sqrtf(ss / (float)K + eps);
}
__device__ __forceinline__ float kon_factor_and_slices(const KonTail& kt, const QMVArgs& a, const float* red, uint32_t n_waves, uint32_t lane) {
    const uint32_t col = lane & 15;
    float inv = 1.0f;
    if (kt.inv_known) {
        inv = kt.inv_pre;
    } else if (kt.prenorm) {
        float s4 = (kt.pp[0] + kt.pp[1]) + (kt.pp[2] + kt.pp[3]);
        for (uint32_t j = lane + 256; j < a.pro.n_ssq; j += 64) s4 += a.pro.ssq[j];
        const float ss = rows_sum4(row16_sum(s4));
        inv = 1.0f / sqrtf(ss / (float)kt.K + kt.eps);
    } else if (kt.norm) {
        const float sv = red[kMaxWaves * 16 + min(col, n_waves - 1)];
        const float ss = row16_sum(col < n_waves ? sv : 0.f);
        inv = 1.0f / sqrtf(ss / (float)kt.K + kt.eps);
    }
    if (kt.has_pro && lane < 16) {
        const QmvPrologue& pr = a.pro;
        if (kt.slice <= 16) {
            const uint32_t k = kt.k0 + lane;
            if (lane < kt.slice && k < kt.K) {
                const float mid = kt.norm ? kt.a_s * inv : kt.a_s;
                if (kt.norm && pr.store_mid) pr.store_mid[k] = mid;
                if (pr.store_x) pr.store_x[k] = mid * kt.b_s;
            }
        } else {
            for (uint32_t k = kt.k0 + lane; k < min(kt.k0 + kt.slice, kt.K); k += 16) {
                const float mid = kt.norm ? pr.a[k] * inv : pr.a[k];
                if (kt.norm && pr.store_mid) pr.store_mid[k] = mid;
                if (pr.store_x) pr.store_x[k] = mid * pr.b[k];
            }
        }
    }
    return inv;
}
template <bool GROUPED, bool KON = false>
__device__ __forceinline__ void reduce_store(float acc, float* red, const QMVArgs& a, uint32_t pi, float* out0, uint32_t g, uint32_t m,
                                             float pre0, bool have_pre0, uint32_t n_waves, const QmvPublish* pub = nullptr, const KonTail* kon = nullptr,
                                             float pre_g = 0.f) {
    const uint32_t lane = threadIdx.x & 63, w = __builtin_amdgcn_readfirstlane(threadIdx.x >> 6);
    if (!KON) {
        acc = rows_sum4(acc);
        if (lane < 16) red[w * 16 + lane] = acc;
    }
    uint32_t kind = kEpiGeneric;
    float ones = 0.f;
    if (GROUPED) {
        kind = pi == 1 ? a.parts[1].epi_kind : pi == 2 ? a.parts[2].epi_kind : pi == 3 ? a.parts[3].epi_kind : a.parts[0].epi_kind;
        if (kind == kEpiSilu && w == 0) {
            const float* const ones_p = pi == 1 ? a.parts[1].epi[2].operand : pi == 2 ? a.parts[2].epi[2].operand : pi == 3 ? a.parts[3].epi[2].operand : a.parts[0].epi[2].operand;
            ones = ones_p[g * 16 + (lane & 15)];
        }
    }
    __syncthreads();
    if (w != 0) return;
    const uint32_t r = lane >> 4, col = lane & 15;
    float part[4];
#pragma unroll
    for (uint32_t j = 0; j < 4; j++) part[j] = red[min(r + 4 * j, n_waves - 1) * 16 + col];
    float v = 0.f;
#pragma unroll
    for (uint32_t j = 0; j < 4; j++) v += r + 4 * j < n_waves ? part[j] : 0.f;
    v = rows_sum4(v);
    if (KON) v *= kon->post * kon_factor_and_slices(*kon, a, red, n_waves, lane);
    if (!KON && kon) v *= kon_factor_and_slices(*kon, a, red, n_waves, lane);
    if (lane < 16) {
        const uint32_t n = g * 16 + threadIdx.x;
        float* out = out0;
        if (GROUPED) out = pi == 1 ? a.parts[1].out : pi == 2 ? a.parts[2].out : pi == 3 ? a.parts[3].out : out;
        float* out_row = out;
        if (m) {
            uint32_t out_rs = a.parts[0].out_rs;
            if (GROUPED) out_rs = pi == 1 ? a.parts[1].out_rs : pi == 2 ? a.parts[2].out_rs : pi == 3 ? a.parts[3].out_rs : out_rs;
            out_row = out + (uint64_t)m * out_rs;
        }
        if (pub)
            __hip_atomic_store((__attribute__((address_space(1))) float*)out_row + n, v, __ATOMIC_RELAXED, __HIP_MEMORY_SCOPE_AGENT);
        else
            out_row[n] = v;
        if (GROUPED && kind == kEpiSilu) {
            if (pi == 0)
                run_epilogue_silu(a.parts[0], n, v, ones);
            else if (pi == 1)
                run_epilogue_silu(a.parts[1], n, v, ones);
            else if (pi == 2)
                run_epilogue_silu(a.parts[2], n, v, ones);
            else
                run_epilogue_silu(a.parts[3], n, v, ones);
        } else if (!GROUPED && have_pre0 && a.parts[0].epi_kind == kEpiResidual) {
            const float h = v + pre0;
            a.parts[0].epi[0].store[n] = h;
            if (a.next.xg_out) {
                a.next.xg_out[n] = h * pre_g;
                const float sq = row16_sum(h * h);
                if (lane == 0) a.next.ssq_out[g] = sq;
            }
        } else if (!GROUPED && have_pre0 && a.parts[0].epi_kind == kEpiMulVec) {
            a.parts[0].epi[0].store[n] = v * pre0;
        } else if (!GROUPED || pi == 0)
            run_epilogue(a.parts[0], n, v, out_row, pre0, !GROUPED && have_pre0);
        else if (pi == 1)
            run_epilogue(a.parts[1], n, v, out_row);
        else if (pi == 2)
            run_epilogue(a.parts[2], n, v, out_row);
        else
            run_epilogue(a.parts[3], n, v, out_row);
    }
    if (pub) {
#if defined(__HIP_DEVICE_COMPILE__)
        asm volatile("s_waitcnt vmcnt(0)" ::: "memory");
#endif
        if (lane == 0 && !(pub->drop && pi == 0 && g == 0))
            __hip_atomic_fetch_add((__attribute__((address_space(1))) uint32_t*)pub->cnt + 32 * (pub->base[pi < 3 ? pi : 2] + (g >> pub->groups_shift)), 1u,
                                   __ATOMIC_RELAXED, __HIP_MEMORY_SCOPE_AGENT);
    }
}



struct XDirect {
    const float* a;
    const float* b;
    float* store_x;
    float* store_mid;
    uint32_t K;
    float inv;
    bool norm;
    __device__ __forceinline__ float pro_value(float av, float bv, uint32_t k, bool live) const {
        float v = av;
        if (norm) {
            v = av * inv;
            if (store_mid && live) store_mid[k] = v;
        }
        v = v * bv;
        if (store_x && live) store_x[k] = v;
        return v;
    }
};

struct SumsqRegs {
    float4 v[4];
};
__device__ __forceinline__ SumsqRegs sumsq_fetch(const float* x, uint32_t K, bool vec, uint32_t T) {
    SumsqRegs r;
    if (vec) {
#pragma unroll
        for (int j = 0; j < 4; j++) {
            const uint32_t k = 4 * (threadIdx.x + j * T);
            r.v[j] = *(const float4*)(x + (k < K ? k : 0));
        }
    } else {
#pragma unroll
        for (int j = 0; j < 4; j++) r.v[j] = make_float4(x[min(threadIdx.x + j * T, K - 1)], 0.f, 0.f, 0.f);
    }
    return r;
}
__device__ __forceinline__ float block_sumsq_direct(const SumsqRegs& r, const float* x, uint32_t K, float* red, bool vec, uint32_t T) {
    float s[4] = {0.f, 0.f, 0.f, 0.f};
    if (vec) {
#pragma unroll
        for (int j = 0; j < 4; j++) {
            const float4 v = r.v[j];
            if (4 * (threadIdx.x + j * T) < K) s[j] += (v.x * v.x + v.y * v.y) + (v.z * v.z + v.w * v.w);
        }
        for (uint32_t k = 4 * threadIdx.x + 16 * T; k < K; k += 4 * T) {
            const float4 v = *(const float4*)(x + k);
            s[0] += (v.x * v.x + v.y * v.y) + (v.z * v.z + v.w * v.w);
        }
    } else {
#pragma unroll
        for (int j = 0; j < 4; j++)
            if (threadIdx.x + j * T < K) s[j] += r.v[j].x * r.v[j].x;
        for (uint32_t k = threadIdx.x + 4 * T; k < K; k += T) s[0] += x[k] * x[k];
    }
    return block_total((s[0] + s[1]) + (s[2] + s[3]), red, T);
}

template <typename ST, int DEPTH, bool XD, bool PROMUL, bool NT>
struct Q4Group {
    uint4 wq[DEPTH];
    Pair<ST> s2[DEPTH];
    float xa[XD ? DEPTH : 1], xb[XD ? DEPTH : 1], ya[XD && PROMUL ? DEPTH : 1], yb[XD && PROMUL ? DEPTH : 1];
    template <int WHAT = 0>
    __device__ __forceinline__ void load(const uint4* qs, const Pair<ST>* sc, uint32_t u, uint32_t stride, uint32_t u_last,
                                         const XDirect& xd, uint32_t i) {
#pragma unroll
        for (int d = 0; d < DEPTH; d++) {
            const uint32_t ud = min(u + d * stride, u_last);
            if (XD && WHAT != 1) {
                const uint32_t ka = min(ud * 32 + i, xd.K - 1), kb = min(ud * 32 + 16 + i, xd.K - 1);
                xa[d] = xd.a[ka], xb[d] = xd.a[kb];
                if (PROMUL) ya[d] = xd.b[ka], yb[d] = xd.b[kb];
            }
            wq[d] = wload<NT>(qs + (uint64_t)ud * 16);
            s2[d] = sc[(uint64_t)ud * 16];
        }
    }
// ... 98 lines not shown
    const uint32_t NB2_0 = nb2_0_flags & 0xFFFFFu, n_parts = (nb2_0_flags >> 24) & 0xF, NB2_1 = nb2_12 & 0xFFFFu, NB2_2 = nb2_12 >> 16;
    uint32_t NB2 = NB2_0, block_begin = 0;
    if (GROUPED && !PAIR) {
        if ((nb2_0_flags >> 28) & 1) {
            const uint32_t b1 = NB2_0, b2 = b1 + NB2_1;
            if (n_parts > 1 && bx >= b1) pi = 1, block_begin = b1, NB2 = NB2_1;
            if (n_parts > 2 && bx >= b2) pi = 2, block_begin = b2, NB2 = NB2_2;
            qs_base = qs0 + (uint64_t)block_begin * U * 16;
            sc_base = (const ScaleT*)sc0 + (uint64_t)(block_begin >> 1) * U * 16;
        } else {
#pragma unroll
            for (uint32_t t = 1; t < (uint32_t)kMaxQmvParts; t++) {
                const bool take = t < n_parts && bx >= a.parts[t].block_begin;
                pi = take ? t : pi;
                qs_base = take ? a.parts[t].qs : qs_base;
                sc_base = take ? a.parts[t].sc : sc_base;
                NB2 = take ? a.parts[t].NB2 : NB2;
                block_begin = take ? a.parts[t].block_begin : block_begin;
            }
        }
    }
    const uint32_t g = column_group(bx - block_begin, NB2), m = blockIdx.y;
    const uint32_t lane = threadIdx.x & 63, w = threadIdx.x >> 6;
    const uint32_t row = lane >> 4, i = lane & 15;
    const uint32_t stride = n_waves * 4;
    const uint4* qs = qs_base + (uint64_t)g * U * 16 + i;
    const ScaleT* sc = (const ScaleT*)sc_base + (uint64_t)(g >> 1) * U * 16 + i;
    const uint32_t n_groups = (U + stride * DEPTH - 1) / (stride * DEPTH);
    const uint32_t u_last = U - 1;

    const float* xa_row = xa_base + (uint64_t)m * in_rs;
    uint32_t u = 4 * w + row;
    const bool pro_owner = XD && PRO && bx == 0 && blockIdx.y == 0;
    XDirect xd{xa_row, xb_base, nullptr, nullptr, K, 1.0f, false};
    Group cur;
    const uint4* const qs_b = qs + (uint64_t)NB2_0 * U * 16;
    const ScaleT* const sc_b = sc + (uint64_t)(NB2_0 >> 1) * U * 16;
    Group cur_b;
    const bool norm = PRO && ((nb2_0_flags >> 29) & 1) != 0;
    const bool x_vec = ((nb2_0_flags >> 30) & 1) != 0;
    float pn_pp[4] = {0.f, 0.f, 0.f, 0.f}, pn_inv = 1.0f;
    if (XD) {
        SumsqRegs sq;
        if (norm) sq = sumsq_fetch(xa_row, K, x_vec, bdim);
        if (PROM == 2) {
            const uint32_t n_ssq = K >> 4;
            const float* const ssq = xa_base + K;
#pragma unroll
            for (uint32_t j = 0; j < 4; j++) {
                const uint32_t q = lane + 64 * j;
                const float v = ssq[min(q, n_ssq - 1)];
                pn_pp[j] = q < n_ssq ? v : 0.f;
            }
        }
        cur.load(qs, sc, u, stride, u_last, xd, i);
        if (PAIR) cur_b.template load<1>(qs_b, sc_b, u, stride, u_last, xd, i);
        QMV_STAMP(1);
        __builtin_amdgcn_sched_barrier(0);
        if (PROM == 2) pn_inv = prenorm_factor(pn_pp, K, a.pro.eps);
        if (pro_owner) xd.store_x = a.pro.store_x, xd.store_mid = a.pro.store_mid;
        if (norm) {
            const float ss = block_sumsq_direct(sq, xa_row, K, red, x_vec, bdim);
            xd.inv = 1.0f / sqrtf(ss / (float)K + a.pro.eps);
            xd.norm = true;
        }
        QMV_STAMP(2);
        QMV_STAMP(3);
    } else {
        const XRegs xa = x_fetch<XVEC>(xa_row, K, bdim);
        const XRegs xb = PRO ? x_fetch<XVEC>(xb_base, K, bdim) : xa;
        cur.load(qs, sc, u, stride, u_last, xd, i);
        QMV_STAMP(1);
        float inv = 1.0f;
        if (norm) {
            const float ss = block_sumsq(xa, K, red, bdim);
            inv = 1.0f / sqrtf(ss / (float)K + a.pro.eps);
        }
        QMV_STAMP(2);
        x_commit<XVEC, PRO>(xs, xa, xb, a.pro, inv, U * UNIT_X, K, xa_row, bdim);
        __syncthreads();
        QMV_STAMP(3);
    }

    uint32_t arg_touch = 0;
#if defined(__HIP_DEVICE_COMPILE__)
    {
        const auto kargs = (const __attribute__((address_space(4))) uint32_t*)__builtin_amdgcn_kernarg_segment_ptr();
        constexpr uint32_t kArgDwords = (56 + sizeof(QMVArgs)) / 4;
#pragma unroll
        for (uint32_t o = 16; o < kArgDwords; o += 16) arg_touch |= kargs[o];
    }
#endif
    KonTail ptail{1.0f, true, 0.f, K, 0.f, 0.f, 16u * bx, 16u, true, true, {0.f, 0.f, 0.f, 0.f}};
    if (PROM == 2) {
        const uint32_t ks = min(ptail.k0 + i, K - 1);
        ptail.a_s = xb_base[ks];
        ptail.b_s = a.pro.b[ks];
        ptail.has_pro = ptail.k0 < K && blockIdx.y == 0;
        ptail.inv_known = !(nb2_0_flags >> 31), ptail.inv_pre = pn_inv;
        ptail.eps = a.pro.eps;
#pragma unroll
        for (uint32_t j = 0; j < 4; j++) ptail.pp[j] = pn_pp[j];
    }
    float pre0 = 0.f, pre_g = 0.f;
    bool have_pre0 = false;
    if (!GROUPED) {
        const float* const op0 = a.parts[0].epi[0].operand;
        have_pre0 = m == 0 && a.parts[0].n_epi != 0 && op0 != nullptr && op0 != out0;
        pre0 = (have_pre0 ? op0 : xa_row)[have_pre0 ? g * 16 + i : 0];
        const float* const gp = a.next.xg_out ? a.next.gamma : nullptr;
        pre_g = (gp ? gp : xa_row)[gp ? g * 16 + i : 0];
    }
    float acc0 = 0.f, acc1 = 0.f, acc2 = 0.f, acc3 = 0.f;
    float bcc0 = 0.f, bcc1 = 0.f, bcc2 = 0.f, bcc3 = 0.f;
    float ones = 0.f;
    if (PAIR) ones = a.parts[0].epi[2].operand[g * 16 + i];
    auto pair_x = [&](Group& b, const Group& src) {
        if constexpr (PAIR) {
#pragma unroll
            for (int d = 0; d < DEPTH; d++) b.xa[d] = src.xa[d], b.xb[d] = src.xb[d];
        }
    };
    for (uint32_t gi = 1; gi < n_groups; gi++) {
        Group nxt, nxt_b;
        nxt.load(qs, sc, u + DEPTH * stride, stride, u_last, xd, i);
        if (PAIR) nxt_b.template load<1>(qs_b, sc_b, u + DEPTH * stride, stride, u_last, xd, i);
        cur.compute(xs, u, stride, U, i, acc0, acc1, acc2, acc3, xd);
        if (PAIR) {
            pair_x(cur_b, cur);
            cur_b.compute(xs, u, stride, U, i, bcc0, bcc1, bcc2, bcc3, xd);
            cur_b = nxt_b;
        }
        cur = nxt;
        u += DEPTH * stride;
    }
    cur.compute(xs, u, stride, U, i, acc0, acc1, acc2, acc3, xd);
    if (PAIR) {
        pair_x(cur_b, cur);
        cur_b.compute(xs, u, stride, U, i, bcc0, bcc1, bcc2, bcc3, xd);
    }
#if defined(__HIP_DEVICE_COMPILE__)
    asm volatile("" ::"s"(arg_touch));
#endif
    QMV_STAMP(4);
    if constexpr (PAIR) {
        const float va = rows_sum4((acc0 + acc1) + (acc2 + acc3)), vb = rows_sum4((bcc0 + bcc1) + (bcc2 + bcc3));
        if (lane < 16) red[w * 16 + lane] = va, red[(kMaxWaves + 1 + w) * 16 + lane] = vb;
        if (PROM != 2) ptail.has_pro = false, ptail.norm = false, ptail.prenorm = false;
        __syncthreads();
        if (w == 0) kon_pair_finish(red, a, out0, g, n_waves, ptail, ones);
    } else {
        reduce_store<GROUPED>((acc0 + acc1) + (acc2 + acc3), red, a, pi, out0, g, m, pre0, have_pre0, n_waves, pub, PROM == 2 ? &ptail : nullptr, pre_g);
    }
    QMV_STAMP(5);
#undef QMV_STAMP
}

template <typename ST, bool XVEC, int DEPTH, bool Q4, bool PRO, bool GROUPED, bool XD, bool NT>
__global__ void __launch_bounds__(1024) qmatvec_kernel(QMV_HEAD_PARAMS, QMVArgs a) {
    qmatvec_body<ST, XVEC, DEPTH, Q4, PRO, GROUPED, XD, NT>(qs0, sc0, out0, xa_base, xb_base, in_rs, K, nb2_0_flags, nb2_12, a, blockIdx.x, nullptr);
}

template <int DEPTH, bool GROUPED>
__global__ void __launch_bounds__(1024) qmatvec_prenorm_kernel(QMV_HEAD_PARAMS, QMVArgs a) {
    qmatvec_body<__half, false, DEPTH, true, 2, GROUPED, true, false>(qs0, sc0, out0, xa_base, xb_base, in_rs, K, nb2_0_flags, nb2_12, a, blockIdx.x, nullptr);
}

template <int DEPTH, int PROM>
__global__ void __launch_bounds__(1024) qmatvec_pair_kernel(QMV_HEAD_PARAMS, QMVArgs a) {
    qmatvec_body<__half, false, DEPTH, true, PROM, true, true, false, true>(qs0, sc0, out0, xa_base, xb_base, in_rs, K, nb2_0_flags, nb2_12, a, blockIdx.x, nullptr);
}

template <bool NT, bool PRO, bool XV, bool PAIR>
struct KonItem {
    uint4 wq, wq_b;
    uint32_t s2, s2_b;
    f32x2 xa, xb;
    __device__ __forceinline__ void load(const uint4* qs, const uint32_t* sc, const float* a, const float* b, uint32_t p, uint32_t p_last, uint32_t K,
                                         uint64_t pair_q, uint64_t pair_s) {
        const uint32_t pd = min(p, p_last);
        if (XV) {
            xa = *(const f32x2*)(a + 2 * pd);
            if (PRO) xb = *(const f32x2*)(b + 2 * pd);
        } else {
            const uint32_t k1 = min(2 * pd + 1, K - 1);
            xa = f32x2{a[2 * pd], a[k1]};
            if (PRO) xb = f32x2{b[2 * pd], b[k1]};
        }
        s2 = sc[pd];
        if (PAIR) s2_b = sc[pair_s + pd];
        wq = wload<NT>(qs + pd);
        if (PAIR) wq_b = wload<NT>(qs + pair_q + pd);
    }
    __device__ __forceinline__ void compute(uint32_t pd, uint32_t P, uint32_t K, f32x2 (&acc)[8], f32x2 (&acc_b)[8], float& T, float& T_b, float& SS) const {
        const bool ok0 = pd < P, ok1 = ok0 && (XV || 2 * pd + 1 < K);
        float x0 = ok0 ? xa.x : 0.f, x1 = ok1 ? xa.y : 0.f;
        if (PRO) {
            SS += x0 * x0;
            SS += x1 * x1;
            x0 *= xb.x, x1 *= xb.y;
        }
        const __half2 h = *(const __half2*)&s2;
        const float t0 = __low2float(h) * x0, t1 = __high2float(h) * x1;
        T += t0;
        T += t1;
        kon_dword(acc, 0, wq.x, t0);
        kon_dword(acc, 4, wq.y, t0);
        kon_dword(acc, 0, wq.z, t1);
        kon_dword(acc, 4, wq.w, t1);
        if (PAIR) {
            const __half2 hb = *(const __half2*)&s2_b;
            const float u0 = __low2float(hb) * x0, u1 = __high2float(hb) * x1;
            T_b += u0;
            T_b += u1;
            kon_dword(acc_b, 0, wq_b.x, u0);
            kon_dword(acc_b, 4, wq_b.y, u0);
            kon_dword(acc_b, 0, wq_b.z, u1);
            kon_dword(acc_b, 4, wq_b.w, u1);
        }
    }
};

__device__ __forceinline__ void kon_pair_finish(const float* red, const QMVArgs& a, float* out0, uint32_t g, uint32_t n_waves, const KonTail& kt, float ones) {
    const uint32_t lane = threadIdx.x & 63, r = lane >> 4, col = lane & 15;
    float pa[4], pb[4];
#pragma unroll
    for (uint32_t j = 0; j < 4; j++) {
        const uint32_t ww = min(r + 4 * j, n_waves - 1);
        pa[j] = red[ww * 16 + col], pb[j] = red[(kMaxWaves + 1 + ww) * 16 + col];
    }
    float va = 0.f, vb = 0.f;
#pragma unroll
    for (uint32_t j = 0; j < 4; j++) va += r + 4 * j < n_waves ? pa[j] : 0.f, vb += r + 4 * j < n_waves ? pb[j] : 0.f;
    va = rows_sum4(va), vb = rows_sum4(vb);
    const float f = kt.post * kon_factor_and_slices(kt, a, red, n_waves, lane);
    va *= f, vb *= f;
    if (lane < 16) {
        const uint32_t n = g * 16 + lane;
        out0[n] = va;
        a.parts[1].out[n] = vb;
        const float e = expf(-va);
        a.parts[0].epi[1].store[n] = e;
        const float sl = (1.0f / (e + ones)) * va;
        a.parts[0].epi[4].store[n] = sl;
        a.pair_out[n] = sl * vb;
    }
}

template <int DEPTH, int PROM, bool GROUPED, bool XV, bool NT, bool PAIR = false>
__device__ __forceinline__ void qmatvec_kon_body(QMV_HEAD_PARAMS, const QMVArgs& a, const uint32_t bx, const uint32_t n_blocks, const QmvPublish* pub) {
    constexpr bool PRO = PROM == 1;
    extern __shared__ float smem[];
    float* red = smem;
#ifdef ZGML_TRACE
#define QMV_STAMP(i) do { if (a.trace && (bx == 0 || bx == n_blocks - 1) && threadIdx.x == 0) a.trace[(bx ? 8 : 0) + i] = wall_clock64(); } while (0)
#else
#define QMV_STAMP(i) do { } while (0)
#endif
    QMV_STAMP(0);
    const uint32_t P = (K + 1) >> 1;
    uint32_t pi = 0;
    const uint4* qs_base = qs0;
    const uint32_t* sc_base = (const uint32_t*)sc0;
    const uint32_t n_waves = ((nb2_0_flags >> 20) & 0xFu) + 1, stride = n_waves * 64;
    const uint32_t NB2_0 = nb2_0_flags & 0xFFFFFu, n_parts = (nb2_0_flags >> 24) & 0xF, NB2_1 = nb2_12 & 0xFFFFu, NB2_2 = nb2_12 >> 16;
    uint32_t NB2 = NB2_0, block_begin = 0;
    if (GROUPED && !PAIR) {
        if ((nb2_0_flags >> 28) & 1) {
            const uint32_t b1 = NB2_0, b2 = b1 + NB2_1;
            if (n_parts > 1 && bx >= b1) pi = 1, block_begin = b1, NB2 = NB2_1;
            if (n_parts > 2 && bx >= b2) pi = 2, block_begin = b2, NB2 = NB2_2;
            qs_base = qs0 + (uint64_t)block_begin * P;
            sc_base = (const uint32_t*)sc0 + (uint64_t)(block_begin >> 1) * P;
        } else {
#pragma unroll
            for (uint32_t t = 1; t < (uint32_t)kMaxQmvParts; t++) {
                const bool take = t < n_parts && bx >= a.parts[t].block_begin;
                pi = take ? t : pi;
                qs_base = take ? a.parts[t].qs : qs_base;
                sc_base = take ? (const uint32_t*)a.parts[t].sc : sc_base;
                NB2 = take ? a.parts[t].NB2 : NB2;
                block_begin = take ? a.parts[t].block_begin : block_begin;
            }
        }
    }
    const uint32_t g = column_group(bx - block_begin, NB2);
    const uint32_t lane = threadIdx.x & 63, w = threadIdx.x >> 6, r = lane >> 4, i = lane & 15;
    const uint4* qs = qs_base + (uint64_t)g * P;
    const uint32_t* sc = sc_base + (uint64_t)(g >> 1) * P;
    const uint32_t n_groups = (P + stride * DEPTH - 1) / (stride * DEPTH), p_last = P - 1;
    const bool norm = PROM == 2 || (PRO && ((nb2_0_flags >> 29) & 1) != 0);
    uint32_t p = threadIdx.x;
    const uint64_t pair_q = PAIR ? (uint64_t)NB2_0 * P : 0, pair_s = PAIR ? (uint64_t)(NB2_0 >> 1) * P : 0;
    KonItem<NT, PRO, XV, PAIR> it[DEPTH];
    float pn_pp[4] = {0.f, 0.f, 0.f, 0.f};
    if (PROM == 2) {
        const uint32_t n_ssq = K >> 4;
#pragma unroll
        for (uint32_t j = 0; j < 4; j++) {
            const uint32_t q = lane + 64 * j;
            const float v = (xa_base + K)[min(q, n_ssq - 1)];
            pn_pp[j] = q < n_ssq ? v : 0.f;
        }
    }
#pragma unroll
    for (int d = 0; d < DEPTH; d++) it[d].load(qs, sc, xa_base, xb_base, p + d * stride, p_last, K, pair_q, pair_s);
    KonTail tail{512.0f, norm, 0.f, K, 0.f, 0.f, 0u, 0u, PROM != 0, PROM == 2, {0.f, 0.f, 0.f, 0.f}};
    if (PROM != 0) {
        tail.slice = (K + n_blocks - 1) / n_blocks;
        tail.k0 = bx * tail.slice;
        const uint32_t ks = min(tail.k0 + i, K - 1);
        tail.a_s = (PROM == 2 ? xb_base : xa_base)[ks];
        tail.b_s = (PROM == 2 ? a.pro.b : xb_base)[ks];
    }
    if (PROM == 2) {
#pragma unroll
        for (uint32_t j = 0; j < 4; j++) tail.pp[j] = pn_pp[j];
    }
    QMV_STAMP(1);
    QMV_STAMP(2);
    QMV_STAMP(3);
    __builtin_amdgcn_sched_barrier(0);
    if (PROM == 2 && (K >> 4) <= 256 && !(nb2_0_flags >> 31))
        tail.inv_pre = prenorm_factor(pn_pp, K, a.pro.eps), tail.inv_known = true;
    uint32_t arg_touch = 0;
#if defined(__HIP_DEVICE_COMPILE__)
    {
        const auto kargs = (const __attribute__((address_space(4))) uint32_t*)__builtin_amdgcn_kernarg_segment_ptr();
        constexpr uint32_t kArgDwords = (56 + sizeof(QMVArgs)) / 4;
#pragma unroll
        for (uint32_t o = 16; o < kArgDwords; o += 16) arg_touch |= kargs[o];
    }
#endif
    float pre0 = 0.f, pre_g = 0.f;
    bool have_pre0 = false;
    if (!GROUPED) {
        const float* const op0 = a.parts[0].epi[0].operand;
        have_pre0 = a.parts[0].n_epi != 0 && op0 != nullptr && op0 != out0;
        pre0 = (have_pre0 ? op0 : xa_base)[have_pre0 ? g * 16 + i : 0];
        const float* const gp = a.next.xg_out ? a.next.gamma : nullptr;
        pre_g = (gp ? gp : xa_base)[gp ? g * 16 + i : 0];
    }
    float ones = 0.f;
    if (PAIR) ones = a.parts[0].epi[2].operand[g * 16 + i];
    f32x2 acc[8], acc_b[PAIR ? 8 : 1];
#pragma unroll
    for (int c = 0; c < 8; c++) acc[c] = f32x2{0.f, 0.f};
#pragma unroll
    for (int c = 0; c < (PAIR ? 8 : 1); c++) acc_b[c] = f32x2{0.f, 0.f};
    float T = 0.f, T_b = 0.f, SS = 0.f;
    auto compute = [&](const KonItem<NT, PRO, XV, PAIR>& item, uint32_t pd) {
        if constexpr (PAIR)
            item.compute(pd, P, K, acc, acc_b, T, T_b, SS);
        else
            item.compute(pd, P, K, acc, acc, T, T_b, SS);
    };
    for (uint32_t gi = 1; gi < n_groups; gi++) {
#pragma unroll
        for (int d = 0; d < DEPTH; d++) {
            compute(it[d], p + d * stride);
            __builtin_amdgcn_sched_barrier(0);
            it[d].load(qs, sc, xa_base, xb_base, p + (DEPTH + d) * stride, p_last, K, pair_q, pair_s);
            __builtin_amdgcn_sched_barrier(0);
        }
        p += DEPTH * stride;
    }
#pragma unroll
    for (int d = 0; d < DEPTH; d++) compute(it[d], p + d * stride);
#if defined(__HIP_DEVICE_COMPILE__)
    asm volatile("" ::"s"(arg_touch));
#endif
    QMV_STAMP(4);
    kon_fold_wave(acc, T, red + w * 16, r, i);
    if constexpr (PAIR) kon_fold_wave(acc_b, T_b, red + (kMaxWaves + 1 + w) * 16, r, i);
    if (PRO) {
        SS = row16_sum(SS);
        SS = kon_fold32(SS, SS);
        SS = kon_fold16(SS, SS);
        if (lane == 0) red[kMaxWaves * 16 + w] = SS;
    }
    if (PROM != 0) tail.eps = a.pro.eps;
    if constexpr (PAIR) {
        __syncthreads();
        if (w == 0) kon_pair_finish(red, a, out0, g, n_waves, tail, ones);
    } else {
        reduce_store<GROUPED, true>(0.f, red, a, pi, out0, g, 0, pre0, have_pre0, n_waves, pub, &tail, pre_g);
    }
    QMV_STAMP(5);
#undef QMV_STAMP
}

template <int DEPTH, int PROM, bool GROUPED, bool XV, bool NT>
__global__ void __launch_bounds__(1024) qmatvec_kon_kernel(QMV_HEAD_PARAMS, QMVArgs a) {
    qmatvec_kon_body<DEPTH, PROM, GROUPED, XV, NT>(qs0, sc0, out0, xa_base, xb_base, in_rs, K, nb2_0_flags, nb2_12, a, blockIdx.x, gridDim.x, nullptr);
}
template <int DEPTH, int PROM, bool NT>
__global__ void __launch_bounds__(512, 4) qmatvec_kon_pair_kernel(QMV_HEAD_PARAMS, QMVArgs a) {
    qmatvec_kon_body<DEPTH, PROM, true, true, NT, true>(qs0, sc0, out0, xa_base, xb_base, in_rs, K, nb2_0_flags, nb2_12, a, blockIdx.x, gridDim.x, nullptr);
}

struct QkvAttnArgs {
    const AttnDecodeParams* params;
    float* split_buf;
    uint32_t* split_cnt;
    uint32_t split_min_keys, n_mv, n_sp;
    uint32_t kvq;
    QmvPublish pub;
    DecodeHandoff ho;
    uint32_t* census;
};
template <typename ST, bool Q4, int LPK, bool KVQ, int PROM = 1>
__global__ void __launch_bounds__(1024) qkv_attn_kernel(QMV_HEAD_PARAMS, QMVArgs a, QkvAttnArgs f) {
    constexpr int DEPTH = 1;
    if (blockIdx.x < f.n_mv) {
        const uint32_t n_waves = ((nb2_0_flags >> 20) & 0xFu) + 1;
        if (threadIdx.x >= n_waves * 64) return;
        qmatvec_body<ST, false, DEPTH, Q4, PROM, true, true, false>(qs0, sc0, out0, xa_base, xb_base, in_rs, K, nb2_0_flags, nb2_12, a, blockIdx.x, &f.pub);
    } else {
        const uint32_t b = blockIdx.x - f.n_mv, n_heads = f.ho.n_heads;
        attention_decode_body<LPK, KVQ>(f.params, f.split_buf, f.split_cnt, f.split_min_keys, b % n_heads, b / n_heads, f.n_sp, &f.ho);
    }
}

template <int LPK, int DEPTH, int PROM, bool NT, bool KVQ, bool CENSUS = false>
__global__ void __launch_bounds__(256, 4) qkv_attn_kon_kernel(QMV_HEAD_PARAMS, QMVArgs a, QkvAttnArgs f) {
    if (CENSUS && f.census) {
        if (threadIdx.x == 0) {
            using gu32c = __attribute__((address_space(1))) uint32_t;
            __hip_atomic_fetch_add((gu32c*)f.census, 1u, __ATOMIC_RELAXED, __HIP_MEMORY_SCOPE_AGENT);
            const uint64_t t0 = __builtin_amdgcn_s_memrealtime();
            while (__hip_atomic_load((gu32c*)f.census, __ATOMIC_RELAXED, __HIP_MEMORY_SCOPE_AGENT) < gridDim.x) {
                if (__builtin_amdgcn_s_memrealtime() - t0 > 20000u) {
                    __hip_atomic_store((gu32c*)f.census + 1, 1u, __ATOMIC_RELAXED, __HIP_MEMORY_SCOPE_AGENT);
                    break;
                }
                __builtin_amdgcn_s_sleep(8);
            }
        }
        return;
    }
    if (blockIdx.x < f.n_mv) {
        qmatvec_kon_body<DEPTH, PROM, true, true, NT>(qs0, sc0, out0, xa_base, xb_base, in_rs, K, nb2_0_flags, nb2_12, a, blockIdx.x, f.n_mv, &f.pub);
    } else {
        const uint32_t b = blockIdx.x - f.n_mv, n_heads = f.ho.n_heads;
        attention_decode_body<LPK, KVQ, 256>(f.params, f.split_buf, f.split_cnt, f.split_min_keys, b % n_heads, b / n_heads, f.n_sp, &f.ho);
    }
}

__device__ __forceinline__ int synth_q4(uint64_t flat, uint32_t id) {
    return (int)((flat * 7 + (flat >> 5) * 3 + (uint64_t)id * 5) & 15) - 8;
}
__device__ __forceinline__ int synth_q8(uint64_t flat, uint32_t id) {
    return (int)((flat * 13 + (uint64_t)id * 29) % 255) - 127;
}
__device__ __forceinline__ float synth_scale(uint64_t block, uint32_t id) {
    return 0.015625f * (1.0f + (float)((block + id) % 7) * 0.125f);
}

__global__ void __launch_bounds__(kBlock) classify_kernel(const int8_t* __restrict__ data, uint64_t n_elems,
                                                          const float* __restrict__ scales, uint64_t n_blocks,
                                                          uint32_t* flags) {
    bool bad_q = false, bad_s = false;
    const uint64_t stride = (uint64_t)gridDim.x * kBlock, t0 = (uint64_t)blockIdx.x * kBlock + threadIdx.x;
    for (uint64_t i = t0; i < n_elems; i += stride) bad_q |= data[i] < -8 || data[i] > 7;
    for (uint64_t b = t0; b < n_blocks; b += stride) bad_s |= __half2float(__float2half_rn(scales[b])) != scales[b];
    if (__any(bad_q) && (threadIdx.x & 63) == 0) atomicOr(&flags[0], 1u);
    if (__any(bad_s) && (threadIdx.x & 63) == 0) atomicOr(&flags[1], 1u);
}

template <typename ST, typename Src>
__device__ __forceinline__ void write_packed(const QWeightDev& w, const Src& src) {
    const uint32_t NB = w.N / 32, NB2 = w.N / 16;
    const bool q4 = w.format == QW_Q4;
    const uint32_t U = q4 ? w.KC : 2 * w.KC;
    const uint64_t n_items = (uint64_t)NB2 * U * 16;
    for (uint64_t it = (uint64_t)blockIdx.x * kBlock + threadIdx.x; it < n_items; it += (uint64_t)gridDim.x * kBlock) {
        const uint32_t i = it & 15;
        const uint64_t gu = it >> 4;
        const uint32_t u = gu % U, g = gu / U;
        const uint32_t n = g * 16 + i;
        uint32_t d[4];
        for (int dd = 0; dd < 4; dd++) {
            uint32_t word = 0;
            for (int b = 0; b < 4; b++) {
                if (q4) {
                    const uint32_t k_lo = u * 32 + 8 * dd + b, k_hi = k_lo + 4;
                    const uint32_t lo = k_lo < w.K ? (uint32_t)src.q(k_lo, n) & 15u : 0u;
                    const uint32_t hi = k_hi < w.K ? (uint32_t)src.q(k_hi, n) & 15u : 0u;
                    word |= (lo | (hi << 4)) << (8 * b);
                } else {
                    const uint32_t k = u * 16 + 4 * dd + b;
                    const uint32_t q = k < w.K ? (uint32_t)src.q(k, n) & 255u : 0u;
                    word |= q << (8 * b);
                }
            }
            d[dd] = word;
        }
        ((uint4*)w.qs)[it] = make_uint4(d[0], d[1], d[2], d[3]);
        if ((g & 1) == 0) {
            const uint32_t j = g >> 1;
            const uint64_t ju = (uint64_t)j * U + u;
            if (q4) {
                const uint32_t ka = u * 32 + i, kb = ka + 16;
                const float sa = ka < w.K ? src.scale(ka, j, NB) : 0.f;
                const float sb = kb < w.K ? src.scale(kb, j, NB) : 0.f;
                ((Pair<ST>*)w.sc)[ju * 16 + i] = Pair<ST>{ST(sa), ST(sb)};
            } else {
                const uint32_t k = u * 16 + i;
                ((ST*)w.sc)[ju * 16 + i] = ST(k < w.K ? src.scale(k, j, NB) : 0.f);
            }
        }
    }
}

template <typename Src>
__device__ __forceinline__ void write_packed_kon(const QWeightDev& w, const Src& src) {
    const uint32_t NB = w.N / 32, NB2 = w.N / 16, P = (w.K + 1) / 2;
    const uint64_t n_items = (uint64_t)NB2 * P;
    for (uint64_t it = (uint64_t)blockIdx.x * kBlock + threadIdx.x; it < n_items; it += (uint64_t)gridDim.x * kBlock) {
        const uint32_t pp = it % P, g = it / P;
        uint32_t d[4];
        for (int dd = 0; dd < 4; dd++) {
            const uint32_t k = 2 * pp + (dd >> 1), c0 = 16 * g + 8 * (dd & 1);
            uint32_t word = 0;
            for (int b = 0; b < 4; b++) {
                const uint32_t lo = k < w.K ? (uint32_t)(src.q(k, c0 + b) + 8) & 15u : 8u;
                const uint32_t hi = k < w.K ? (uint32_t)(src.q(k, c0 + 4 + b) + 8) & 15u : 8u;
                word |= (lo | (hi << 4)) << (8 * b);
// ... 168 lines not shown
}

bool launch_packed(hipStream_t s, QMVArgs& a, const QWeightDev& w0, uint32_t total_blocks, uint32_t M, bool xvec, const QkvAttnArgs* fused = nullptr,
                   uint32_t extra_blocks = 0, uint32_t d_head = 0);
static uint32_t head_flags(const QMVArgs& a, uint32_t waves, bool contig, bool rmsnorm, bool late) {
    return a.parts[0].NB2 | ((waves - 1) << 20) | (a.n_parts << 24) | (contig ? 1u << 28 : 0u) | (rmsnorm ? 1u << 29 : 0u) | (a.x_vec ? 1u << 30 : 0u) | (late ? 1u << 31 : 0u);
}

uint32_t kon_waves(const QWeightDev& w) {
    const uint32_t wave_steps = cdiv((w.K + 1) / 2, 64);
    const int big_cap = sw().qmv_kon_waves > 0 ? sw().qmv_kon_waves : (w.K > 6144 ? 8 : 4);
    const uint32_t cap = (uint32_t)std::max(1, std::min(16, w.K <= 2048 ? sw().qmv_kon_waves_smallk : big_cap));
    return std::max(1u, std::min(wave_steps, cap));
}

template <int PROM, bool GRP, bool XV>
KernelFn pick_kon_depth(int depth_sel, bool nt) {
    switch (depth_sel) {
        case 0: return qmatvec_kon_kernel<1, PROM, GRP, XV, false>;
        case 1: return qmatvec_kon_kernel<2, PROM, GRP, XV, false>;
        default:
            if constexpr (PROM == 1)
                return qmatvec_kon_kernel<2, PROM, GRP, XV, false>;
            else
                return nt ? qmatvec_kon_kernel<4, PROM, GRP, XV, true> : qmatvec_kon_kernel<4, PROM, GRP, XV, false>;
    }
}
template <int PROM>
KernelFn pick_kon_mode(bool grp, bool xv, int depth_sel, bool nt) {
    if (xv) return grp ? pick_kon_depth<PROM, true, true>(depth_sel, nt) : pick_kon_depth<PROM, false, true>(depth_sel, nt);
    return grp ? pick_kon_depth<PROM, true, false>(depth_sel, nt) : pick_kon_depth<PROM, false, false>(depth_sel, nt);
}
KernelFn pick_kon(int prom, bool grp, bool xv, int depth_sel, bool nt) {
    if (prom == 2) return pick_kon_mode<2>(grp, xv, depth_sel, nt);
    if (prom == 1) return pick_kon_mode<1>(grp, xv, depth_sel, nt);
    return pick_kon_mode<0>(grp, xv, depth_sel, nt);
}

bool launch_packed_kon(hipStream_t s, QMVArgs& a, const QWeightDev& w0, uint32_t total_blocks, bool xvec, const QkvAttnArgs* fused, uint32_t extra_blocks,
                       uint32_t d_head) {
    a.x_vec = xvec ? 1 : 0;
    const uint32_t P = (a.K + 1) / 2;
    uint32_t waves = kon_waves(w0);
    int tune_depth = 0;
    {
        for (const char* q = sw().qmv_kon_tune; q && *q;) {
            unsigned b = 0, k = 0, wv = 0, dp = 0;
            const int got = sscanf(q, "%ux%u:%u:%u", &b, &k, &wv, &dp);
            if (got >= 3 && b == total_blocks && k == a.K && wv >= 1 && wv <= 16) {
                waves = wv;
                if (got == 4) tune_depth = (int)dp;
            }
            q = strchr(q, ',');
            if (q) q++;
        }
    }
    bool contig = a.n_parts > 1 && a.n_parts <= 3 && sw().qmv_contig;
    for (uint32_t t = 1; t < a.n_parts && contig; t++) {
        const QMVPartDev &pv = a.parts[t - 1], &pt = a.parts[t];
        contig = (const char*)pt.qs == (const char*)pv.qs + (size_t)pv.NB2 * P * 16 && (const char*)pt.sc == (const char*)pv.sc + (size_t)(pv.NB2 / 2) * P * 4 &&
                 pt.block_begin == pv.block_begin + pv.NB2;
    }
    if (a.n_parts > 1 && (a.parts[1].NB2 > 0xFFFFu || (a.n_parts > 2 && a.parts[2].NB2 > 0xFFFFu))) contig = false;
    const uint32_t nb2_12 = contig ? (a.parts[1].NB2 | (a.n_parts > 2 ? a.parts[2].NB2 << 16 : 0u)) : 0u;
    const size_t lds = ((size_t)kMaxWaves * 16 + kMaxWaves) * sizeof(float);
    const bool pro = a.pro.kind != QMV_PRO_NONE, grp = a.n_parts > 1, nt = w0.stream_nt != 0;
    const int prom = a.pro.kind == QMV_PRO_PRENORM ? 2 : (pro ? 1 : 0);
    if (prom == 2 && a.pro.ssq != a.pro.xg + a.K) {
        fprintf(stderr, "[zgml_hip] ERROR: a PRENORM launch whose partial sums do not follow its vector: not launched\n");
        return false;
    }
    uint32_t waves_used = waves;
    if (prom == 1 && cdiv(P, waves * 64) >= 4) waves_used = std::min<uint32_t>(kMaxWaves, waves * 2);
    const uint32_t n_steps = cdiv(P, waves_used * 64);
    int depth_sel = n_steps >= 4 ? 2 : (n_steps >= 2 ? 1 : 0);
    if (tune_depth == 4) depth_sel = 2;
    if (tune_depth == 2) depth_sel = 1;
    if (prom == 1 && depth_sel >= 2) depth_sel = 1;
    const float* const head_xa = prom == 2 ? a.pro.xg : a.pro.a;
    const float* const head_xb = prom == 2 ? a.pro.a : a.pro.b;
    const uint32_t flags = head_flags(a, waves_used, contig, a.pro.kind == QMV_PRO_RMSNORM_MUL, sw().hip_prenorm_early == 0);
    if (fused) {
        using FusedFn = void (*)(const uint4*, const void*, float*, const float*, const float*, uint32_t, uint32_t, uint32_t, uint32_t, QMVArgs, QkvAttnArgs);
        if (!grp || !contig || !xvec || prom == 1 || (d_head != 64 && d_head != 128)) return false;
        const uint32_t steps4 = cdiv(P, 4 * 64);
        const bool deep = steps4 >= 4;
        const uint32_t flags4 = (flags & ~(0xFu << 20)) | (3u << 20);
        FusedFn ff = nullptr;
#define ZGML_QKV_KON(LPK_, KVQ_)                                                                                                                   \
    ff = prom == 2 ? (deep ? (nt ? qkv_attn_kon_kernel<LPK_, 4, 2, true, KVQ_> : qkv_attn_kon_kernel<LPK_, 4, 2, false, KVQ_>) : qkv_attn_kon_kernel<LPK_, 2, 2, false, KVQ_>) \
                   : (deep ? (nt ? qkv_attn_kon_kernel<LPK_, 4, 0, true, KVQ_> : qkv_attn_kon_kernel<LPK_, 4, 0, false, KVQ_>) : qkv_attn_kon_kernel<LPK_, 2, 0, false, KVQ_>)
        if (d_head == 64) {
            if (fused->kvq) ZGML_QKV_KON(16, true); else ZGML_QKV_KON(16, false);
        } else {
            if (fused->kvq) ZGML_QKV_KON(32, true); else ZGML_QKV_KON(32, false);
        }
#undef ZGML_QKV_KON
        QkvAttnArgs f = *fused;
        f.n_mv = total_blocks;
        hipLaunchKernelGGL(ff, dim3(total_blocks + extra_blocks), dim3(256), lds, s, a.parts[0].qs, a.parts[0].sc, a.parts[0].out, head_xa, head_xb, a.in_rs, a.K, flags4, nb2_12,
                           a, f);
        return true;
    }
    if (a.pair_out) {
        const bool pair_ok = a.n_parts == 2 && contig && xvec && prom != 1 && a.parts[0].NB2 == a.parts[1].NB2 && a.parts[0].NB2 % 2 == 0 && waves_used <= 8;
        if (!pair_ok) {
            fprintf(stderr, "[zgml_hip] ERROR: a gate / up pair launch that does not meet the pair kernel's layout conditions: not launched\n");
            return false;
        }
        using PairFn = void (*)(const uint4*, const void*, float*, const float*, const float*, uint32_t, uint32_t, uint32_t, uint32_t, QMVArgs);
        PairFn pf = nullptr;
        if (prom == 2)
            pf = depth_sel == 0 ? qmatvec_kon_pair_kernel<1, 2, false> : (nt ? qmatvec_kon_pair_kernel<2, 2, true> : qmatvec_kon_pair_kernel<2, 2, false>);
        else
            pf = depth_sel == 0 ? qmatvec_kon_pair_kernel<1, 0, false> : (nt ? qmatvec_kon_pair_kernel<2, 0, true> : qmatvec_kon_pair_kernel<2, 0, false>);
        const size_t lds2 = ((size_t)(2 * kMaxWaves + 1) * 16) * sizeof(float);
        hipLaunchKernelGGL(pf, dim3(a.parts[0].NB2), dim3(waves_used * 64), lds2, s, a.parts[0].qs, a.parts[0].sc, a.parts[0].out, head_xa, head_xb, a.in_rs, a.K, flags, nb2_12, a);
        return true;
    }
    const KernelFn fn = pick_kon(prom, grp, xvec, depth_sel, nt);
    hipLaunchKernelGGL(fn, dim3(total_blocks), dim3(waves_used * 64), lds, s, a.parts[0].qs, a.parts[0].sc, a.parts[0].out, head_xa, head_xb, a.in_rs, a.K, flags, nb2_12, a);
    return true;
}

bool launch_packed(hipStream_t s, QMVArgs& a, const QWeightDev& w0, uint32_t total_blocks, uint32_t M, bool xvec, const QkvAttnArgs* fused,
                   uint32_t extra_blocks, uint32_t d_head) {
    if (sw().hip_debug_skip_grid && total_blocks == (uint32_t)sw().hip_debug_skip_grid) return true;
    if (w0.format == QW_Q4K) {
        if (M != 1) return false;
        return launch_packed_kon(s, a, w0, total_blocks, xvec, fused, extra_blocks, d_head);
    }
    const bool q4 = w0.format == QW_Q4;
    a.x_vec = xvec ? 1 : 0;
    const bool xd = sw().qmv_xdirect && (a.pro.kind != QMV_PRO_RMSNORM_MUL || (sw().qmv_xdirect_norm && a.K <= (uint32_t)sw().qmv_xdnorm_maxk));
    const bool prenorm = a.pro.kind == QMV_PRO_PRENORM;
    if (prenorm && (!qmv_prenorm_ok(w0, a.K, total_blocks * 16, M) || a.pro.ssq != a.pro.xg + a.K)) {
        fprintf(stderr, "[zgml_hip] ERROR: a PRENORM mat-vec launch outside the shapes its kernel is built for: not launched\n");
        return false;
    }
    uint32_t waves = qmv_waves(w0);
    if (!xd && a.pro.kind != QMV_PRO_NONE)
        while (waves < (uint32_t)kMaxWaves && waves * 64 * 4 * kXRegs < a.K) waves++;
    bool contig = a.n_parts > 1 && a.n_parts <= 3 && sw().qmv_contig;
    const size_t sc_elem = (q4 ? 2 : 1) * (w0.scale_f16 ? 2 : 4);
    for (uint32_t t = 1; t < a.n_parts && contig; t++) {
        const QMVPartDev &pv = a.parts[t - 1], &pt = a.parts[t];
        contig = (const char*)pt.qs == (const char*)pv.qs + (size_t)pv.NB2 * a.U * 256 &&
                 (const char*)pt.sc == (const char*)pv.sc + (size_t)(pv.NB2 / 2) * a.U * 16 * sc_elem &&
                 pt.block_begin == pv.block_begin + pv.NB2;
    }
    dim3 grid(total_blocks, M);
    const size_t lds = xd ? (size_t)kMaxWaves * 16 * sizeof(float) : qmv_lds_bytes(w0);
    const uint32_t n_steps = cdiv(a.U, waves * 4);
    const int depth_sel = n_steps >= 4 ? 2 : (n_steps >= 2 ? 1 : 0);
    const bool pro = a.pro.kind == QMV_PRO_MUL || a.pro.kind == QMV_PRO_RMSNORM_MUL, grp = a.n_parts > 1;
    const bool nt = w0.stream_nt != 0;
    const float* const head_xa = prenorm ? a.pro.xg : a.pro.a;
    const float* const head_xb = prenorm ? a.pro.a : a.pro.b;
    const bool rmsnorm = a.pro.kind == QMV_PRO_RMSNORM_MUL, late = sw().hip_prenorm_early == 0;
    const KernelFn fn = prenorm ? (grp ? (depth_sel == 0 ? qmatvec_prenorm_kernel<1, true> : depth_sel == 1 ? qmatvec_prenorm_kernel<2, true> : qmatvec_prenorm_kernel<4, true>)
                                       : (depth_sel == 0 ? qmatvec_prenorm_kernel<1, false> : depth_sel == 1 ? qmatvec_prenorm_kernel<2, false> : qmatvec_prenorm_kernel<4, false>))
                      : w0.scale_f16 ? pick_kernel<__half>(xvec, q4, pro, grp, depth_sel, xd, nt)
                                     : pick_kernel<float>(xvec, q4, pro, grp, depth_sel, xd, nt);
    if (lds > 64 * 1024)
        hipFuncSetAttribute((const void*)fn, hipFuncAttributeMaxDynamicSharedMemorySize, (int)kMaxLds);
    if (a.n_parts > 1 && (a.parts[1].NB2 > 0xFFFFu || (a.n_parts > 2 && a.parts[2].NB2 > 0xFFFFu))) contig = false;
    const uint32_t nb2_12 = contig ? (a.parts[1].NB2 | (a.n_parts > 2 ? a.parts[2].NB2 << 16 : 0u)) : 0u;
    if (a.pair_out) {
        const bool pair_ok = qmv_pair_ok(w0) && xd && !pro && !fused && a.n_parts == 2 && contig && M == 1 && a.parts[0].NB2 == a.parts[1].NB2 && a.parts[0].NB2 % 2 == 0;
        if (!pair_ok) {
            fprintf(stderr, "[zgml_hip] ERROR: a gate / up pair launch that does not meet the pair kernel's layout conditions: not launched\n");
            return false;
        }
        const KernelFn pf = prenorm ? (depth_sel == 0 ? qmatvec_pair_kernel<1, 2> : depth_sel == 1 ? qmatvec_pair_kernel<2, 2> : qmatvec_pair_kernel<4, 2>)
                                    : (depth_sel == 0 ? qmatvec_pair_kernel<1, 0> : depth_sel == 1 ? qmatvec_pair_kernel<2, 0> : qmatvec_pair_kernel<4, 0>);
        const size_t lds2 = ((size_t)(2 * kMaxWaves + 1) * 16) * sizeof(float);
        hipLaunchKernelGGL(pf, dim3(a.parts[0].NB2), dim3(waves * 64), lds2, s, a.parts[0].qs, a.parts[0].sc, a.parts[0].out, head_xa, head_xb, a.in_rs, a.K,
                           head_flags(a, waves, true, false, late), nb2_12, a);
        return true;
    }
    if (fused) {
        if (!(xd && (pro || prenorm) && grp && !nt && q4 && w0.scale_f16 && contig && M == 1 && a.n_parts == 3 && (d_head == 64 || d_head == 128))) return false;
        QkvAttnArgs f = *fused;
        f.n_mv = total_blocks;
        const bool fused_kvq = f.kvq != 0;
        if (depth_sel != 0) return false;
        using FusedFn = void (*)(const uint4*, const void*, float*, const float*, const float*, uint32_t, uint32_t, uint32_t, uint32_t, QMVArgs, QkvAttnArgs);
        FusedFn ff = nullptr;
        if (d_head == 64)
            ff = prenorm ? (fused_kvq ? qkv_attn_kernel<__half, true, 16, true, 2> : qkv_attn_kernel<__half, true, 16, false, 2>)
                         : (fused_kvq ? qkv_attn_kernel<__half, true, 16, true> : qkv_attn_kernel<__half, true, 16, false>);
        else
            ff = prenorm ? (fused_kvq ? qkv_attn_kernel<__half, true, 32, true, 2> : qkv_attn_kernel<__half, true, 32, false, 2>)
                         : (fused_kvq ? qkv_attn_kernel<__half, true, 32, true> : qkv_attn_kernel<__half, true, 32, false>);
        hipLaunchKernelGGL(ff, dim3(total_blocks + extra_blocks), dim3(1024), lds, s, a.parts[0].qs, a.parts[0].sc, a.parts[0].out, head_xa, head_xb, a.in_rs, a.K,
                           head_flags(a, waves, true, rmsnorm, late), nb2_12, a, f);
        return true;
    }
    hipLaunchKernelGGL(fn, grid, dim3(waves * 64), lds, s, a.parts[0].qs, a.parts[0].sc, a.parts[0].out, head_xa, head_xb, a.in_rs, a.K,
                       head_flags(a, waves, contig, rmsnorm, late), nb2_12, a);
    return true;
}

}

uint32_t qmv_max_prologue_k(const QWeightDev& w) { return w.format == QW_Q4K ? UINT32_MAX : kMaxWaves * 64 * 4 * kXRegs; }

void launch_qmatvec_rows(hipStream_t s, const QWeightDev& w, const QMatmulParams& p, bool xvec) {
    QMVArgs a{};
    a.n_parts = 1;
    a.parts[0].qs = (const uint4*)w.qs;
    a.parts[0].sc = w.sc;
    a.parts[0].out = p.dst;
    a.parts[0].NB2 = p.N / 16;
    a.parts[0].block_begin = 0;
    a.parts[0].out_rs = p.dst_rs;
    a.parts[0].n_epi = 0;
    a.pro.kind = QMV_PRO_NONE;
    a.pro.a = p.input;
    a.pro.b = p.input;
    a.M = p.M, a.K = p.K;
    a.U = w.format == QW_Q4 ? w.KC : 2 * w.KC;
    a.in_rs = p.in_rs;
    a.trace = nullptr;
    launch_packed(s, a, w, a.parts[0].NB2, p.M, xvec);
}

static void build_qmv_args(const QmvLaunch& L, QMVArgs& a, uint32_t& blocks, bool& xvec_out) {
    const QWeightDev& w0 = L.parts[0].w;
    a = QMVArgs{};
    a.n_parts = L.n_parts;
    blocks = 0;
    for (uint32_t i = 0; i < L.n_parts; i++) {
        const QmvPart& pt = L.parts[i];
        QMVPartDev& d = a.parts[i];
        d.qs = (const uint4*)pt.w.qs;
        d.sc = pt.w.sc;
        d.out = pt.dst;
        d.NB2 = pt.w.N / 16;
        d.block_begin = blocks;
        d.out_rs = pt.w.N;
        d.n_epi = pt.n_epi;
        for (uint32_t e = 0; e < pt.n_epi; e++) d.epi[e] = pt.epi[e];
        {
            const QmvEpiStep* st = pt.epi;
            const bool silu = pt.n_epi == 5 && st[0].op == ZGML_OP_NEG && !st[0].store && st[1].op == ZGML_OP_EXP && st[1].store &&
                              st[2].op == ZGML_OP_ADD && st[2].operand && st[2].operand != pt.dst && st[2].operand != st[1].store && !st[2].store &&
                              st[3].op == ZGML_OP_RECIP && !st[3].store && st[4].op == ZGML_OP_MUL && st[4].operand == pt.dst && st[4].store;
            const bool residual = pt.n_epi == 1 && st[0].op == ZGML_OP_ADD && st[0].operand && st[0].operand != pt.dst && st[0].store;
            const bool mulvec = pt.n_epi == 1 && st[0].op == ZGML_OP_MUL && st[0].operand && st[0].operand != pt.dst && st[0].store;
            d.epi_kind = silu ? (sw().qmv_epi_silu ? kEpiSilu : kEpiGeneric) : (residual ? kEpiResidual : (mulvec ? kEpiMulVec : kEpiGeneric));
        }
        blocks += d.NB2;
    }
    a.pro = L.pro;
    a.next = L.next;
    a.pair_out = L.pair_out;
    if (a.pro.kind == QMV_PRO_NONE) a.pro.b = a.pro.a;
    a.M = 1, a.K = L.K;
    a.U = w0.format == QW_Q4 ? w0.KC : 2 * w0.KC;
    a.in_rs = L.K;
    bool xvec = ((uintptr_t)L.pro.a % 16 == 0) && (L.K % 4 == 0);
    if (L.pro.kind != QMV_PRO_NONE) xvec = xvec && ((uintptr_t)L.pro.b % 16 == 0);
    if (L.pro.kind == QMV_PRO_PRENORM) xvec = xvec && ((uintptr_t)L.pro.xg % 16 == 0);
    a.trace = L.trace;
    xvec_out = xvec;
}

static bool launch_qmv(hipStream_t s, const QmvLaunch& L, const QkvAttnArgs* fused, uint32_t extra_blocks, uint32_t d_head) {
    if (L.n_parts == 0) return false;
    QMVArgs a;
    uint32_t blocks = 0;
    bool xvec = false;
    build_qmv_args(L, a, blocks, xvec);
    return launch_packed(s, a, L.parts[0].w, blocks, 1, xvec, fused, extra_blocks, d_head);
}

void launch_qmatvec_fused(hipStream_t s, const QmvLaunch& L) { launch_qmv(s, L, nullptr, 0, 0); }

bool launch_qkv_attention(hipStream_t s, const QmvLaunch& L, const AttnDecodeParams* dev_params, uint32_t n_heads, uint32_t n_kv, uint32_t d_head,
                          const AttnSplit& sp, uint32_t* counters, const uint32_t* idx, uint32_t* seen, uint32_t* timeout, bool kvq) {
    QkvAttnArgs f{};
    f.kvq = kvq ? 1 : 0;
    f.params = dev_params, f.split_buf = sp.buf, f.split_cnt = sp.cnt, f.split_min_keys = sp.min_keys;
    f.n_sp = sp.splits ? sp.splits : 1;
    uint32_t shift = 0;
    while ((16u << shift) < d_head) shift++;
    f.pub = QmvPublish{counters, {0, n_heads, n_heads + n_kv}, shift, sw().hip_debug_drop_publish ? 1u : 0u};
    f.ho = DecodeHandoff{counters, seen, idx, n_heads, d_head / 16, timeout, (uint32_t)sw().hip_handoff_sleep};
    return launch_qmv(s, L, &f, n_heads * f.n_sp, d_head);
}

int qkv_attn_kon_census(hipStream_t s, uint32_t d_head, bool kvq, uint32_t grid) {
    using Fn = void (*)(const uint4*, const void*, float*, const float*, const float*, uint32_t, uint32_t, uint32_t, uint32_t, QMVArgs, QkvAttnArgs);
    const Fn census = d_head == 64 ? (kvq ? (Fn)qkv_attn_kon_kernel<16, 4, 2, true, true, true> : (Fn)qkv_attn_kon_kernel<16, 4, 2, true, false, true>)
                                   : (kvq ? (Fn)qkv_attn_kon_kernel<32, 4, 2, true, true, true> : (Fn)qkv_attn_kon_kernel<32, 4, 2, true, false, true>);
    const Fn product = d_head == 64 ? (kvq ? (Fn)qkv_attn_kon_kernel<16, 4, 2, true, true> : (Fn)qkv_attn_kon_kernel<16, 4, 2, true, false>)
                                    : (kvq ? (Fn)qkv_attn_kon_kernel<32, 4, 2, true, true> : (Fn)qkv_attn_kon_kernel<32, 4, 2, true, false>);
    hipFuncAttributes fa{}, fb{};
    if (hipFuncGetAttributes(&fa, (const void*)census) != hipSuccess || hipFuncGetAttributes(&fb, (const void*)product) != hipSuccess) return -1;
    if (fa.numRegs < fb.numRegs || fa.sharedSizeBytes != fb.sharedSizeBytes) return -1;
    uint32_t* blk = nullptr;
    if (hipMalloc((void**)&blk, 8) != hipSuccess) return -1;
    int result = -1;
    uint32_t host[2] = {0, 1};
    if (hipMemsetAsync(blk, 0, 8, s) == hipSuccess) {
        QMVArgs a{};
        QkvAttnArgs f{};
        f.census = blk;
        const size_t lds = ((size_t)kMaxWaves * 16 + kMaxWaves) * sizeof(float);
        hipLaunchKernelGGL(census, dim3(grid), dim3(256), lds, s, (const uint4*)nullptr, (const void*)nullptr, (float*)nullptr, (const float*)nullptr, (const float*)nullptr, 0u, 0u, 0u,
                           0u, a, f);
        if (hipMemcpyAsync(host, blk, 8, hipMemcpyDeviceToHost, s) == hipSuccess && hipStreamSynchronize(s) == hipSuccess)
            result = host[0] == grid && host[1] == 0 ? 1 : 0;
    }
    hipFree(blk);
    return result;
}

int qkv_attn_kon_blocks_per_cu(uint32_t d_head, bool kvq) {
    int nb = 0;
    const void* fn = d_head == 64 ? (kvq ? (const void*)qkv_attn_kon_kernel<16, 4, 2, true, true> : (const void*)qkv_attn_kon_kernel<16, 4, 2, true, false>)
                                  : (kvq ? (const void*)qkv_attn_kon_kernel<32, 4, 2, true, true> : (const void*)qkv_attn_kon_kernel<32, 4, 2, true, false>);
    if (hipOccupancyMaxActiveBlocksPerMultiprocessor(&nb, fn, 256, ((size_t)kMaxWaves * 16 + kMaxWaves) * sizeof(float)) != hipSuccess) return 0;
    return nb;
}

void launch_synth_packed(hipStream_t s, const QWeightDev& w, uint32_t matrix_id) {
    if (w.scale_f16)
        synth_packed_kernel<__half><<<2048, kBlock, 0, s>>>(w, matrix_id);
    else
        synth_packed_kernel<float><<<2048, kBlock, 0, s>>>(w, matrix_id);
}

}
```

Before: 1689 tokens/s.

## Replace counter-based QKV→attention handoff with generation-tagged value granules

The fused QKV matvec + attention decode kernel now publishes each projected output as a 64-bit granule that packs the value with a per-block generation number. The attention blocks poll these granules directly into LDS until every generation matches, so they no longer wait on separate per-head counters after a vmcnt drain plus atomic add. This is meant to shorten the producer-to-consumer latency and drop the counter atomics and the extra reload of q/k/v. In exchange it doubles the published bytes, adds generation bookkeeping buffers, and keeps the old counter path only for the kon variant.

```diff
diff --git a/zgml_amd/csrc/attention_decode.h b/zgml_amd/csrc/attention_decode.h
--- a/zgml_amd/csrc/attention_decode.h
+++ b/zgml_amd/csrc/attention_decode.h
@@ -1,6 +1,6 @@
 #pragma once
 #include "kernels.h"
-
+#include "handoff_gen.h"
 #include <hip/hip_fp16.h>
 #include <math.h>
 
@@ -207,19 +207,21 @@
 }
 
 struct DecodeHandoff {
-    const uint32_t* cnt;
-    uint32_t* seen;
-    const uint32_t* idx;
+    const unsigned long long* gran;
+    uint32_t rel[3];
+    uint32_t* gen;
     uint32_t n_heads;
-    uint32_t need;
     uint32_t* timeout;
     uint32_t poll_sleep;
 };
-
-template <int LPK, bool KVQ, int BLOCK = kAttnBlock>
+__device__ __forceinline__ void handoff_idle(const DecodeHandoff* ho, uint32_t wg, uint32_t gen) { ho->gen[wg] = gen; }
+__device__ __forceinline__ void handoff_idle(const CounterHandoff* ho, uint32_t wg, uint32_t) { for (int c = 0; c < 3; c++) ho->seen[3 * wg + c] += ho->need; }
+__device__ __forceinline__ void handoff_done(const DecodeHandoff* ho, uint32_t wg, uint32_t gen, const uint32_t (&)[3]) { ho->gen[wg] = gen; }
+__device__ __forceinline__ void handoff_done(const CounterHandoff* ho, uint32_t wg, uint32_t, const uint32_t (&t)[3]) { for (int c = 0; c < 3; c++) ho->seen[3 * wg + c] = t[c]; }
+template <int LPK, bool KVQ, int BLOCK = kAttnBlock, typename HO = DecodeHandoff>
 __device__ __forceinline__ void attention_decode_body(const AttnDecodeParams* __restrict__ params, float* split_buf, uint32_t* split_cnt,
-                                                      uint32_t split_min_keys, const uint32_t hx, const uint32_t sp_in, const uint32_t n_sp,
-                                                      const DecodeHandoff* ho) {
+                                                      uint32_t split_min_keys, const uint32_t hx, const uint32_t sp_in, const uint32_t n_sp, const HO* ho) {
+    constexpr bool COUNTERS = std::is_same<HO, CounterHandoff>::value;
     constexpr int DH = 4 * LPK, HALF = DH / 2;
     constexpr bool Q16 = KVQ && ZGML_ATTN_KVQ16 != 0 && LPK >= 32;
     constexpr int LPKM = Q16 ? DH / 16 : LPK, KPW = 64 / LPKM, KPW4 = 64 / LPK, U = Q16 ? kAttnUnrollQ16 : kAttnUnroll;
@@ -262,12 +264,13 @@
     constexpr int COLV = DH / 4 + DH / 32;
     __shared__ __attribute__((aligned(16))) float q16_lds[Q16 ? DH : 4];
     __shared__ __attribute__((aligned(16))) uint32_t col_lds[Q16 ? 2 * COLV : 4];
+    __shared__ __attribute__((aligned(16))) float qkv_lds[3 * DH];
     const uint32_t tid = threadIdx.x, lane = tid & 63, w = tid >> 6;
     const uint32_t slot = lane / LPK, li = lane % LPK, d0 = 4 * li, pair = d0 & (HALF - 1);
     const bool is_hi = d0 >= (uint32_t)HALF;
     const uint32_t seq_kv = KVQ ? min(ldgu(p.dyn_seq_kv), P.kvq_cols) : ldgu(p.dyn_seq_kv), dk = ldgu(P.dyn_k_off), dv = ldgu(P.dyn_v_off);
     const uint32_t d2_off = p.dst2 ? ldgu(p.dyn_dst2_off) : 0;
-    const bool wait_qkv = ho && ho->cnt;
+    const bool wait_qkv = ho != nullptr;
     float4 q_own, q_par, k_own, k_par, v_new;
     if (!wait_qkv) {
         q_own = ldg4(P.q_src + d0), q_par = ldg4(P.q_src + (d0 ^ HALF));
@@ -279,14 +282,13 @@
     ATTN_STAMP(1);
     const uint32_t sp = sp_in;
     uint32_t n_active = 1, k_begin = 0, k_end = seq_kv;
+    uint32_t gen = 0;
+    if constexpr (!COUNTERS) gen = wait_qkv ? handoff_next_gen(ho->gen[hx * n_sp + sp]) : 0;
     if (n_sp > 1) {
         n_active = seq_kv / split_min_keys;
         n_active = n_active < 1 ? 1 : (n_active > n_sp ? n_sp : n_active);
         if (sp >= n_active) {
-            if (wait_qkv && tid == 0) {
-                uint32_t* const seen = ho->seen + (hx * n_sp + sp) * 3;
-                seen[0] += ho->need, seen[1] += ho->need, seen[2] += ho->need;
-            }
+            if (wait_qkv && tid == 0) handoff_idle(ho, hx * n_sp + sp, gen);
             return;
         }
         const uint32_t chunk = (seq_kv + n_active - 1) / n_active;
@@ -353,7 +355,7 @@
         }
     }
     uint32_t target[3] = {0, 0, 0};
-    if (wait_qkv) {
+    if constexpr (COUNTERS) {
         const uint32_t ci[3] = {ho->idx[3 * hx], ho->idx[3 * hx + 1], ho->idx[3 * hx + 2]};
         const uint32_t* const seen = ho->seen + (hx * n_sp + sp) * 3;
 #pragma unroll
@@ -384,6 +386,42 @@
         q_own = ld_agent4(P.q_src + d0), q_par = ld_agent4(P.q_src + (d0 ^ HALF));
         k_own = ld_agent4(P.k_src + d0), k_par = ld_agent4(P.k_src + (d0 ^ HALF));
         v_new = ld_agent4(P.v_src + d0);
+    } else if (wait_qkv) {
+        if (w == 0) {
+            constexpr int PER = DH / 64 > 0 ? DH / 64 : 1, NG = 3 * PER;
+            static_assert(DH % 64 == 0 || DH < 64, "a slice is swept by whole waves");
+            typedef const __attribute__((address_space(1))) char* gbytes;
+            const gbytes g0 = (gbytes)ho->gran;
+            const gbytes gs[3] = {g0 + (2u * (uint32_t)(uintptr_t)P.q_src + ho->rel[0]), g0 + (2u * (uint32_t)(uintptr_t)P.k_src + ho->rel[1]),
+                                  g0 + (2u * (uint32_t)(uintptr_t)P.v_src + ho->rel[2])};
+            const bool in_slice = DH >= 64 || lane < (uint32_t)DH;
+            const uint32_t lane8 = in_slice ? 8u * lane : 0u;
+            uint32_t spins = 0;
+            for (;;) {
+                bool ok = true;
+#pragma unroll
+                for (int k = 0; k < NG; k++) {
+                    const unsigned long long x = __hip_atomic_load((const gu64*)(gs[k / PER] + lane8) + 64 * (k % PER), __ATOMIC_RELAXED, __HIP_MEMORY_SCOPE_AGENT);
+                    if (in_slice) qkv_lds[(k / PER) * DH + 64 * (k % PER) + lane] = __uint_as_float(handoff_granule_value(x));
+                    ok = ok && handoff_granule_gen(x) == gen;
+                }
+                if (__builtin_amdgcn_ballot_w64(!ok) == 0) break;
+                if (++spins > 400000u) {
+                    if (tid == 0) __hip_atomic_store(ho->timeout, 1u, __ATOMIC_RELAXED, __HIP_MEMORY_SCOPE_SYSTEM);
+                    break;
+                }
+                for (uint32_t z = 0; z < ho->poll_sleep; z++) __builtin_amdgcn_s_sleep(1);
+            }
+        }
+        __builtin_amdgcn_fence(__ATOMIC_RELEASE, "wavefront");
+        __builtin_amdgcn_wave_barrier();
+#if defined(__HIP_DEVICE_COMPILE__)
+        if (NW > 1) asm volatile("s_waitcnt lgkmcnt(0)\n\ts_barrier" ::: "memory");
+#endif
+        __builtin_amdgcn_fence(__ATOMIC_ACQUIRE, "wavefront");
+        q_own = *(const float4*)&qkv_lds[d0], q_par = *(const float4*)&qkv_lds[d0 ^ HALF];
+        k_own = *(const float4*)&qkv_lds[DH + d0], k_par = *(const float4*)&qkv_lds[DH + (d0 ^ HALF)];
+        v_new = *(const float4*)&qkv_lds[2 * DH + d0];
     }
     ATTN_STAMP(2);
     const float4 qv = rope4(q_own, q_par, q_c, q_s, is_hi);
@@ -593,10 +631,7 @@
         ATTN_STAMP(6);
     }
     {
-        if (wait_qkv && lane == 0) {
-            uint32_t* const seen = ho->seen + (hx * n_sp + sp) * 3;
-            seen[0] = target[0], seen[1] = target[1], seen[2] = target[2];
-        }
+        if (wait_qkv && lane == 0) handoff_done(ho, hx * n_sp + sp, gen, target);
         if (n_active > 1) {
             constexpr uint32_t REC = DH + 4;
             float* const head_buf = split_buf + (uint64_t)hx * n_sp * REC;
@@ -642,8 +677,8 @@
 template <int LPK, bool KVQ, int BLOCK = kAttnBlock>
 __global__ void __launch_bounds__(BLOCK) attention_decode_kernel(const AttnDecodeParams* __restrict__ params, float* split_buf,
                                                                  uint32_t* split_cnt, uint32_t split_min_keys) {
-    attention_decode_body<LPK, KVQ, BLOCK>(params, split_buf, split_cnt, split_min_keys, blockIdx.x, blockIdx.y, gridDim.y, nullptr);
-}
-
-}
-}
+    attention_decode_body<LPK, KVQ, BLOCK>(params, split_buf, split_cnt, split_min_keys, blockIdx.x, blockIdx.y, gridDim.y, (const DecodeHandoff*)nullptr);
+}
+
+}
+}
diff --git a/zgml_amd/csrc/handoff_gen.h b/zgml_amd/csrc/handoff_gen.h
--- /dev/null
+++ b/zgml_amd/csrc/handoff_gen.h
@@ -0,0 +1,34 @@
+#pragma once
+#include <stdint.h>
+#include <type_traits>
+
+#if defined(__HIPCC__) || defined(__CUDACC__)
+#define ZGML_HANDOFF_HD __host__ __device__
+#else
+#define ZGML_HANDOFF_HD
+#endif
+
+namespace zgml {
+
+ZGML_HANDOFF_HD constexpr uint32_t handoff_next_gen(uint32_t g) { return g + 1u ? g + 1u : 1u; }
+
+ZGML_HANDOFF_HD constexpr unsigned long long handoff_granule(uint32_t value_bits, uint32_t gen) {
+    return (unsigned long long)value_bits | ((unsigned long long)gen << 32);
+}
+ZGML_HANDOFF_HD constexpr uint32_t handoff_granule_gen(unsigned long long granule) { return (uint32_t)(granule >> 32); }
+ZGML_HANDOFF_HD constexpr uint32_t handoff_granule_value(unsigned long long granule) { return (uint32_t)granule; }
+
+static_assert(handoff_next_gen(0u) == 1u && handoff_next_gen(0xFFFFFFFEu) == 0xFFFFFFFFu && handoff_next_gen(0xFFFFFFFFu) == 1u,
+              "generations run 1 .. 0xFFFFFFFF and skip 0");
+
+struct CounterHandoff {
+    const uint32_t* cnt;
+    uint32_t* seen;
+    const uint32_t* idx;
+    uint32_t n_heads;
+    uint32_t need;
+    uint32_t* timeout;
+    uint32_t poll_sleep;
+};
+
+}
diff --git a/zgml_amd/csrc/kernels.h b/zgml_amd/csrc/kernels.h
--- a/zgml_amd/csrc/kernels.h
+++ b/zgml_amd/csrc/kernels.h
@@ -523,9 +523,15 @@
 bool qmv_can_group(const QWeightDev& a, const QWeightDev& b);
 uint32_t qmv_max_prologue_k(const QWeightDev& w);
 void launch_qmatvec_fused(hipStream_t s, const QmvLaunch& L);
+struct QkvHandoffBlock {
+    unsigned long long* granules = nullptr;
+    uint32_t *producer_gen = nullptr, *consumer_gen = nullptr;
+    uint32_t* counters = nullptr;
+    const uint32_t* idx = nullptr;
+    uint32_t* seen = nullptr;
+};
 bool launch_qkv_attention(hipStream_t s, const QmvLaunch& L, const AttnDecodeParams* dev_params, uint32_t n_heads, uint32_t n_kv, uint32_t d_head,
-                          const AttnSplit& sp, uint32_t* counters, const uint32_t* idx, uint32_t* seen, uint32_t* timeout,
-                          bool kvq = false);
+                          const AttnSplit& sp, const QkvHandoffBlock& hb, uint32_t* timeout, bool kvq = false);
 int qkv_attn_kon_census(hipStream_t s, uint32_t d_head, bool kvq, uint32_t grid);
 int qkv_attn_kon_blocks_per_cu(uint32_t d_head, bool kvq);
 void launch_synth_packed(hipStream_t s, const QWeightDev& w, uint32_t matrix_id);
diff --git a/zgml_amd/csrc/ksplit.hip b/zgml_amd/csrc/ksplit.hip
--- a/zgml_amd/csrc/ksplit.hip
+++ b/zgml_amd/csrc/ksplit.hip
@@ -203,6 +203,7 @@
     uint32_t base[3];
     uint32_t groups_shift;
 };
+using KsHandoff = CounterHandoff;
 template <int GP, int U>
 __device__ __forceinline__ void ks_proj_body(const KsProjArgs& a, float* smem, const KsPublish* pub) {
     const uint32_t T = a.n_threads ? a.n_threads : blockDim.x, W = T >> 6, b = blockIdx.x;
@@ -366,7 +367,7 @@
 };
 constexpr int kKsAttnBlock = 768;
 template <int LPK, bool KVQ, int UO>
-__device__ __forceinline__ void ks_attn_o_body(const KsAttnArgs& f, const uint32_t hx, const uint32_t sp, const DecodeHandoff* ho) {
+__device__ __forceinline__ void ks_attn_o_body(const KsAttnArgs& f, const uint32_t hx, const uint32_t sp, const KsHandoff* ho) {
     constexpr int DH = 4 * LPK, KPW = 64 / LPK, U = kAttnUnroll, HALF = DH / 2, CH = DH / 32, BLOCK = kKsAttnBlock;
     static_assert(DH % 32 == 0, "the head's rows of W_o are whole 32-k chunks");
     using Row = AttnRow<KVQ>;
@@ -691,7 +692,7 @@
     KsProjArgs pj;
     KsAttnArgs at;
     KsPublish pub;
-    DecodeHandoff ho;
+    KsHandoff ho;
     uint32_t n_proj, n_heads;
     uint32_t dbg;
 };
@@ -862,7 +863,7 @@
     uint32_t shift = 0;
     while ((16u << shift) < AL.d_head) shift++;
     g.pub = KsPublish{counters, {0, AL.n_heads, AL.n_heads + n_kv}, shift};
-    g.ho = DecodeHandoff{counters, seen, idx, AL.n_heads, (AL.d_head / 16) / 2, timeout, (uint32_t)sw().hip_handoff_sleep};
+    g.ho = KsHandoff{counters, seen, idx, AL.n_heads, (AL.d_head / 16) / 2, timeout, (uint32_t)sw().hip_handoff_sleep};
     g.n_proj = wgs, g.n_heads = AL.n_heads;
     g.dbg = (uint32_t)sw().ks_debug_a;
     using Fn = void (*)(KsLayerAArgs);
diff --git a/zgml_amd/csrc/plan.hip b/zgml_amd/csrc/plan.hip
--- a/zgml_amd/csrc/plan.hip
+++ b/zgml_amd/csrc/plan.hip
@@ -583,24 +583,33 @@
             }
             if (it->second == 0) continue;
         }
-        const size_t n_cnt = 32 * ((size_t)nh + 2 * n_kv);
-        const size_t words = n_cnt + (size_t)nh * n_sp * 3 + 1 + 3 * (size_t)nh;
-        uint32_t* block = nullptr;
-        if (hipMalloc((void**)&block, words * 4) != hipSuccess) continue;
-        if (memset_sync(p->ctx->stream, block, 0, words * 4) != hipSuccess) {
+        const size_t n_gran = ((size_t)nh + 2 * n_kv) * dh, n_cnt = 32 * ((size_t)nh + 2 * n_kv);
+        const size_t bytes = kon ? (n_cnt + (size_t)nh * n_sp * 3 + 1 + idx.size()) * 4 : (n_gran * 8 + (n_mv + (size_t)nh * n_sp) * 4 + 15) / 16 * 16;
+        void* block = nullptr;
+        if (hipMalloc(&block, bytes) != hipSuccess) continue;
+        if (memset_sync(p->ctx->stream, block, 0, bytes) != hipSuccess) {
             hipFree(block);
             continue;
         }
         p->fuse_owned.push_back(block);
-        uint32_t *counters = block, *seen = block + n_cnt, *timeout = p->ctx->handoff_flag_dev, *idx_dev = seen + (size_t)nh * n_sp * 3 + 1;
-        if (h2d_sync(p->ctx->stream, idx_dev, idx.data(), idx.size() * 4) != hipSuccess) continue;
+        uint32_t* const timeout = p->ctx->handoff_flag_dev;
+        QkvHandoffBlock hb;
+        if (kon) {
+            hb.counters = (uint32_t*)block, hb.seen = hb.counters + n_cnt;
+            uint32_t* const idx_dev = hb.seen + (size_t)nh * n_sp * 3 + 1;
+            if (h2d_sync(p->ctx->stream, idx_dev, idx.data(), idx.size() * 4) != hipSuccess) continue;
+            hb.idx = idx_dev;
+        } else {
+            hb.granules = (unsigned long long*)block;
+            hb.producer_gen = (uint32_t*)(hb.granules + n_gran), hb.consumer_gen = hb.producer_gen + n_mv;
+        }
         const AttnDecodeParams* d = ad->dev;
         AttnSplit sp = ad->sp;
         sp.splits = n_sp;
         const uint32_t n_ops = p->plan[i].n_ops + p->plan[i + 1].n_ops, lo = std::min(p->plan[i].op_lo, p->plan[i + 1].op_lo),
                        hi = std::max(p->plan[i].op_hi, p->plan[i + 1].op_hi);
         Launch F{ZGML_DOP_QMATMUL, n_ops, lo, hi, [=](hipStream_t s) {
-                     if (!launch_qkv_attention(s, L, d, nh, n_kv, dh, sp, counters, idx_dev, seen, timeout, kvq)) {
+                     if (!launch_qkv_attention(s, L, d, nh, n_kv, dh, sp, hb, timeout, kvq)) {
                          launch_qmatvec_fused(s, L);
                          launch_attention_decode_batch(s, d, nh, dh, sp, kvq);
                      }
diff --git a/zgml_amd/csrc/qmatvec.hip b/zgml_amd/csrc/qmatvec.hip
--- a/zgml_amd/csrc/qmatvec.hip
+++ b/zgml_amd/csrc/qmatvec.hip
@@ -153,6 +153,11 @@
 }
 
 struct QmvPublish {
+    unsigned long long* gran;
+    uint32_t* gen;
+    uint32_t drop;
+};
+struct QmvCountPublish {
     uint32_t* cnt;
     uint32_t base[3];
     uint32_t groups_shift;
@@ -210,10 +215,10 @@
     }
     return inv;
 }
-template <bool GROUPED, bool KON = false>
+template <bool GROUPED, bool KON = false, typename PUB = QmvPublish>
 __device__ __forceinline__ void reduce_store(float acc, float* red, const QMVArgs& a, uint32_t pi, float* out0, uint32_t g, uint32_t m,
-                                             float pre0, bool have_pre0, uint32_t n_waves, const QmvPublish* pub = nullptr, const KonTail* kon = nullptr,
-                                             float pre_g = 0.f) {
+                                             float pre0, bool have_pre0, uint32_t n_waves, const PUB* pub = nullptr, const KonTail* kon = nullptr,
+                                             float pre_g = 0.f, uint32_t pub_cg = 0, uint32_t pub_gen = 0) {
     const uint32_t lane = threadIdx.x & 63, w = __builtin_amdgcn_readfirstlane(threadIdx.x >> 6);
     if (!KON) {
         acc = rows_sum4(acc);
@@ -250,10 +255,17 @@
             if (GROUPED) out_rs = pi == 1 ? a.parts[1].out_rs : pi == 2 ? a.parts[2].out_rs : pi == 3 ? a.parts[3].out_rs : out_rs;
             out_row = out + (uint64_t)m * out_rs;
         }
-        if (pub)
-            __hip_atomic_store((__attribute__((address_space(1))) float*)out_row + n, v, __ATOMIC_RELAXED, __HIP_MEMORY_SCOPE_AGENT);
-        else
+        constexpr bool COUNTERS = std::is_same<PUB, QmvCountPublish>::value;
+        if constexpr (COUNTERS) {
+            if (pub)
+                __hip_atomic_store((__attribute__((address_space(1))) float*)out_row + n, v, __ATOMIC_RELAXED, __HIP_MEMORY_SCOPE_AGENT);
+            else
+                out_row[n] = v;
+        } else {
+            if (pub && !(pub->drop && pub_cg == 0))
+                __hip_atomic_store((gu64*)pub->gran + (pub_cg * 16 + lane), handoff_granule(__float_as_uint(v), pub_gen), __ATOMIC_RELAXED, __HIP_MEMORY_SCOPE_AGENT);
             out_row[n] = v;
+        }
         if (GROUPED && kind == kEpiSilu) {
             if (pi == 0)
                 run_epilogue_silu(a.parts[0], n, v, ones);
@@ -282,13 +294,17 @@
         else
             run_epilogue(a.parts[3], n, v, out_row);
     }
-    if (pub) {
+    if constexpr (std::is_same<PUB, QmvCountPublish>::value) {
+        if (pub) {
 #if defined(__HIP_DEVICE_COMPILE__)
-        asm volatile("s_waitcnt vmcnt(0)" ::: "memory");
+            asm volatile("s_waitcnt vmcnt(0)" ::: "memory");
 #endif
-        if (lane == 0 && !(pub->drop && pi == 0 && g == 0))
-            __hip_atomic_fetch_add((__attribute__((address_space(1))) uint32_t*)pub->cnt + 32 * (pub->base[pi < 3 ? pi : 2] + (g >> pub->groups_shift)), 1u,
-                                   __ATOMIC_RELAXED, __HIP_MEMORY_SCOPE_AGENT);
+            if (lane == 0 && !(pub->drop && pi == 0 && g == 0))
+                __hip_atomic_fetch_add((__attribute__((address_space(1))) uint32_t*)pub->cnt + 32 * (pub->base[pi < 3 ? pi : 2] + (g >> pub->groups_shift)), 1u,
+                                       __ATOMIC_RELAXED, __HIP_MEMORY_SCOPE_AGENT);
+        }
+    } else {
+        if (pub && lane == 0) pub->gen[pub_cg] = pub_gen;
     }
 }
 
@@ -553,6 +569,8 @@
         QMV_STAMP(3);
     }
 
+    uint32_t pub_gen = 0;
+    if (pub) pub_gen = __hip_atomic_load((gu32*)pub->gen + (block_begin + g), __ATOMIC_RELAXED, __HIP_MEMORY_SCOPE_AGENT);
     uint32_t arg_touch = 0;
 #if defined(__HIP_DEVICE_COMPILE__)
     {
@@ -621,7 +639,8 @@
         __syncthreads();
         if (w == 0) kon_pair_finish(red, a, out0, g, n_waves, ptail, ones);
     } else {
-        reduce_store<GROUPED>((acc0 + acc1) + (acc2 + acc3), red, a, pi, out0, g, m, pre0, have_pre0, n_waves, pub, PROM == 2 ? &ptail : nullptr, pre_g);
+        reduce_store<GROUPED>((acc0 + acc1) + (acc2 + acc3), red, a, pi, out0, g, m, pre0, have_pre0, n_waves, pub, PROM == 2 ? &ptail : nullptr, pre_g,
+                             block_begin + g, handoff_next_gen(pub_gen));
     }
     QMV_STAMP(5);
 #undef QMV_STAMP
@@ -719,7 +738,7 @@
 }
 
 template <int DEPTH, int PROM, bool GROUPED, bool XV, bool NT, bool PAIR = false>
-__device__ __forceinline__ void qmatvec_kon_body(QMV_HEAD_PARAMS, const QMVArgs& a, const uint32_t bx, const uint32_t n_blocks, const QmvPublish* pub) {
+__device__ __forceinline__ void qmatvec_kon_body(QMV_HEAD_PARAMS, const QMVArgs& a, const uint32_t bx, const uint32_t n_blocks, const QmvCountPublish* pub) {
     constexpr bool PRO = PROM == 1;
     extern __shared__ float smem[];
     float* red = smem;
@@ -878,6 +897,8 @@
     uint32_t kvq;
     QmvPublish pub;
     DecodeHandoff ho;
+    QmvCountPublish cpub;
+    CounterHandoff cho;
     uint32_t* census;
 };
 template <typename ST, bool Q4, int LPK, bool KVQ, int PROM = 1>
@@ -911,10 +932,10 @@
         return;
     }
     if (blockIdx.x < f.n_mv) {
-        qmatvec_kon_body<DEPTH, PROM, true, true, NT>(qs0, sc0, out0, xa_base, xb_base, in_rs, K, nb2_0_flags, nb2_12, a, blockIdx.x, f.n_mv, &f.pub);
+        qmatvec_kon_body<DEPTH, PROM, true, true, NT>(qs0, sc0, out0, xa_base, xb_base, in_rs, K, nb2_0_flags, nb2_12, a, blockIdx.x, f.n_mv, &f.cpub);
     } else {
-        const uint32_t b = blockIdx.x - f.n_mv, n_heads = f.ho.n_heads;
-        attention_decode_body<LPK, KVQ, 256>(f.params, f.split_buf, f.split_cnt, f.split_min_keys, b % n_heads, b / n_heads, f.n_sp, &f.ho);
+        const uint32_t b = blockIdx.x - f.n_mv, n_heads = f.cho.n_heads;
+        attention_decode_body<LPK, KVQ, 256>(f.params, f.split_buf, f.split_cnt, f.split_min_keys, b % n_heads, b / n_heads, f.n_sp, &f.cho);
     }
 }
 
@@ -1249,7 +1270,7 @@
     const uint32_t flags = head_flags(a, waves_used, contig, a.pro.kind == QMV_PRO_RMSNORM_MUL, sw().hip_prenorm_early == 0);
     if (fused) {
         using FusedFn = void (*)(const uint4*, const void*, float*, const float*, const float*, uint32_t, uint32_t, uint32_t, uint32_t, QMVArgs, QkvAttnArgs);
-        if (!grp || !contig || !xvec || prom == 1 || (d_head != 64 && d_head != 128)) return false;
+        if (!grp || !contig || !xvec || prom == 1 || (d_head != 64 && d_head != 128) || !fused->cho.cnt) return false;
         const uint32_t steps4 = cdiv(P, 4 * 64);
         const bool deep = steps4 >= 4;
         const uint32_t flags4 = (flags & ~(0xFu << 20)) | (3u << 20);
@@ -1347,7 +1368,7 @@
         return true;
     }
     if (fused) {
-        if (!(xd && (pro || prenorm) && grp && !nt && q4 && w0.scale_f16 && contig && M == 1 && a.n_parts == 3 && (d_head == 64 || d_head == 128))) return false;
+        if (!(xd && (pro || prenorm) && grp && !nt && q4 && w0.scale_f16 && contig && M == 1 && a.n_parts == 3 && (d_head == 64 || d_head == 128) && fused->ho.gran)) return false;
         QkvAttnArgs f = *fused;
         f.n_mv = total_blocks;
         const bool fused_kvq = f.kvq != 0;
@@ -1446,15 +1467,26 @@
 void launch_qmatvec_fused(hipStream_t s, const QmvLaunch& L) { launch_qmv(s, L, nullptr, 0, 0); }
 
 bool launch_qkv_attention(hipStream_t s, const QmvLaunch& L, const AttnDecodeParams* dev_params, uint32_t n_heads, uint32_t n_kv, uint32_t d_head,
-                          const AttnSplit& sp, uint32_t* counters, const uint32_t* idx, uint32_t* seen, uint32_t* timeout, bool kvq) {
+                          const AttnSplit& sp, const QkvHandoffBlock& hb, uint32_t* timeout, bool kvq) {
+    if (L.n_parts != 3) return false;
     QkvAttnArgs f{};
     f.kvq = kvq ? 1 : 0;
     f.params = dev_params, f.split_buf = sp.buf, f.split_cnt = sp.cnt, f.split_min_keys = sp.min_keys;
     f.n_sp = sp.splits ? sp.splits : 1;
-    uint32_t shift = 0;
-    while ((16u << shift) < d_head) shift++;
-    f.pub = QmvPublish{counters, {0, n_heads, n_heads + n_kv}, shift, sw().hip_debug_drop_publish ? 1u : 0u};
-    f.ho = DecodeHandoff{counters, seen, idx, n_heads, d_head / 16, timeout, (uint32_t)sw().hip_handoff_sleep};
+    const uint32_t drop = sw().hip_debug_drop_publish ? 1u : 0u;
+    if (hb.counters) {
+        uint32_t shift = 0;
+        while ((16u << shift) < d_head) shift++;
+        f.cpub = QmvCountPublish{hb.counters, {0, n_heads, n_heads + n_kv}, shift, drop};
+        f.cho = CounterHandoff{hb.counters, hb.seen, hb.idx, n_heads, d_head / 16, timeout, (uint32_t)sw().hip_handoff_sleep};
+        return launch_qmv(s, L, &f, n_heads * f.n_sp, d_head);
+    }
+    if (!hb.granules) return false;
+    unsigned long long* const granules = hb.granules;
+    f.pub = QmvPublish{granules, hb.producer_gen, drop};
+    const uint32_t first[3] = {0, n_heads * d_head, (n_heads + n_kv) * d_head};
+    f.ho = DecodeHandoff{granules, {0, 0, 0}, hb.consumer_gen, n_heads, timeout, (uint32_t)sw().hip_handoff_sleep};
+    for (int c = 0; c < 3; c++) f.ho.rel[c] = 8u * first[c] - 2u * (uint32_t)(uintptr_t)L.parts[c].dst;
     return launch_qmv(s, L, &f, n_heads * f.n_sp, d_head);
 }
 
```

Result: faster. 1751 tokens/s (median of 6 runs) (+3.6%).
